# goroda/GPEXP

Hardware: AMD Instinct MI355X
Metric: GP-fit+IVAR-eval points/s at N=32768 d=8 (wall-time in ms_per_step); value = (N+M)/t_step, SURVEY 8d's N/t_fit and M/t_IVAR are points_per_s_fit / points_per_s_ivar right behind it (higher is better)
Workload: dtype f64; 1 GPU; C4: N=32768 d=8 Matern-5/2 (rho=0.5,s=1,noise=0.1) kfill+potrf+potrs+logdet+IVAR over M=32768 MC points; N=32768, d=8, M=32768, kernel=matern52, seed=32768, parallelism=1 GPU

## Files before the change

gpexp_amd/_lib.py:

```python
import ctypes as C
import os

import numpy as np

_HERE = os.path.dirname(os.path.abspath(__file__))
LIB_PATH = os.path.join(_HERE, "libgpx_hip.so")

c_i64 = C.c_int64
c_dp = C.POINTER(C.c_double)
c_ip = C.POINTER(c_i64)
c_vp = C.c_void_p

_SIGS = {
    "gpx_abi_version": (C.c_int, []),
    "gpx_last_error": (C.c_char_p, []),
    "gpx_create": (C.c_int, [C.c_int, C.POINTER(c_vp)]),
    "gpx_destroy": (C.c_int, [c_vp]),
    "gpx_sync": (C.c_int, [c_vp]),
    "gpx_trim": (C.c_int, [c_vp]),
    "gpx_device_info": (C.c_int, [c_vp, C.c_char_p, C.c_int, C.POINTER(C.c_int), c_ip, C.POINTER(C.c_int)]),
    "gpx_mat_from_host": (C.c_int, [c_vp, c_dp, c_i64, c_i64, C.c_int, C.POINTER(c_vp)]),
    "gpx_mat_alloc": (C.c_int, [c_vp, c_i64, c_i64, C.c_int, C.POINTER(c_vp)]),
    "gpx_mat_free": (C.c_int, [c_vp, c_vp]),
    "gpx_mat_clone": (C.c_int, [c_vp, c_vp, C.POINTER(c_vp)]),
    "gpx_mat_shape": (C.c_int, [c_vp, c_ip, c_ip, c_ip]),
    "gpx_mat_to_host": (C.c_int, [c_vp, c_vp, c_dp, C.c_int]),
    "gpx_kfill": (C.c_int, [c_vp, C.c_int, C.c_int, c_dp, C.c_int, c_vp, c_vp, c_dp, c_i64, C.POINTER(c_vp)]),
    "gpx_kfill_into": (C.c_int, [c_vp, C.c_int, C.c_int, c_dp, C.c_int, c_vp, c_vp, c_dp, c_i64, c_vp]),
    "gpx_kdiag": (C.c_int, [c_vp, C.c_int, C.c_int, c_dp, C.c_int, c_vp, c_dp]),
    "gpx_kernel_eval": (C.c_int, [c_vp, C.c_int, C.c_int, c_dp, C.c_int, c_dp, c_i64, c_dp, c_i64, c_dp]),
    "gpx_potrf": (C.c_int, [c_vp, c_vp]),
    "gpx_potrf_policy": (C.c_int, [c_vp, C.c_double, C.c_int]),
    "gpx_potrf_dropped": (C.c_int, [c_vp, C.POINTER(C.c_int)]),
    "gpx_refit_rows": (C.c_int, [c_vp, C.c_int, C.c_int, c_dp, C.c_int, c_vp, c_dp, c_i64, c_vp, c_i64, C.POINTER(c_vp)]),
    "gpx_potrs": (C.c_int, [c_vp, c_vp, c_dp, c_dp]),
    "gpx_col_sumsq": (C.c_int, [c_vp, c_vp, c_i64, c_dp]),
    "gpx_dist_ivar_step": (C.c_int, [c_vp, c_vp, c_i64, c_i64, c_vp]),
    "gpx_dist_ivar_group": (C.c_int, [c_vp, c_vp, c_i64, c_i64, c_i64, c_vp]),
    "gpx_dist_ivar_group_at": (C.c_int, [c_vp, c_vp, c_i64, c_i64, c_i64, c_vp, c_i64]),
    "gpx_dist_fwd_group_at": (C.c_int, [c_vp, c_vp, c_i64, c_i64, c_i64, c_vp, c_i64]),
    "gpx_matvec": (C.c_int, [c_vp, c_vp, c_dp, c_dp]),
    "gpx_fitc_fit": (C.c_int, [c_vp, C.c_int, C.c_int, c_dp, C.c_int, c_vp, c_vp, C.c_double, C.POINTER(c_vp)]),
    "gpx_fitc_free": (C.c_int, [c_vp, c_vp]),
    "gpx_fitc_shape": (C.c_int, [c_vp, C.POINTER(c_i64), C.POINTER(c_i64)]),
    "gpx_fitc_solve": (C.c_int, [c_vp, c_vp, c_dp, c_dp, c_dp]),
    "gpx_fitc_logdet": (C.c_int, [c_vp, c_vp, c_dp]),
    "gpx_fitc_posterior": (C.c_int, [c_vp, c_vp, c_vp, c_dp, c_vp, c_dp, c_dp]),
    "gpx_fitc_dense": (C.c_int, [c_vp, c_vp, c_dp, c_dp]),
    "gpx_potrs_dev": (C.c_int, [c_vp, c_vp, c_vp, c_vp]),
    "gpx_logdet": (C.c_int, [c_vp, c_vp, c_dp]),
    "gpx_potri": (C.c_int, [c_vp, c_vp, C.POINTER(c_vp)]),
    "gpx_posterior": (C.c_int, [c_vp, C.c_int, C.c_int, c_dp, C.c_int, c_vp, c_vp, c_dp, c_vp, c_dp, c_dp]),
    "gpx_posterior_cov": (C.c_int, [c_vp, C.c_int, C.c_int, c_dp, C.c_int, c_vp, c_vp, c_vp, c_dp]),
    "gpx_fit_ivar": (C.c_int, [c_vp, C.c_int, C.c_int, c_dp, C.c_int, c_vp, c_vp, c_vp, c_dp]),
    "gpx_ivar": (C.c_int, [c_vp, C.c_int, C.c_int, c_dp, C.c_int, c_vp, c_vp, c_vp, c_dp]),
    "gpx_ivar_keep": (C.c_int, [c_vp, C.c_int, C.c_int, c_dp, C.c_int, c_vp, c_vp, c_vp, c_dp, C.POINTER(c_vp)]),
    "gpx_ivar_update": (C.c_int, [c_vp, C.c_int, C.c_int, c_dp, C.c_int, c_vp, c_vp, c_vp, c_vp, c_i64, c_dp]),
    "gpx_greedy_var": (C.c_int, [c_vp, C.c_int, C.c_int, c_dp, C.c_int, c_vp, c_dp, c_ip, c_i64, c_i64, c_ip]),
    "gpx_greedy_ivar_step": (C.c_int, [c_vp, C.c_int, C.c_int, c_dp, C.c_int, c_vp, c_vp, c_vp, c_vp,
                                       C.c_double, c_dp, c_ip]),
    "gpx_greedy_ivar": (C.c_int, [c_vp, C.c_int, C.c_int, c_dp, C.c_int, c_vp, c_vp, c_vp, c_vp, C.c_double, c_i64, c_ip, c_dp,
                                  c_dp]),
    "gpx_givar_begin": (C.c_int, [c_vp, C.c_int, C.c_int, c_dp, C.c_int, c_vp, c_vp, c_vp, c_vp, C.c_double, c_i64,
                                  C.POINTER(c_vp)]),
    "gpx_givar_pivot_elems": (c_i64, [c_vp]),
    "gpx_givar_score": (C.c_int, [c_vp, c_vp, c_dp, c_ip, c_dp]),
    "gpx_givar_pack": (C.c_int, [c_vp, c_vp, c_i64, c_vp]),
    "gpx_givar_apply": (C.c_int, [c_vp, c_vp, c_vp]),
    "gpx_givar_end": (C.c_int, [c_vp, c_vp]),
    "gpx_mi_greedy": (C.c_int, [c_vp, C.c_int, C.c_int, c_dp, C.c_int, c_vp, C.c_double, c_i64, c_i64, c_ip, c_dp]),
    "gpx_acq": (C.c_int, [c_vp, C.c_int, C.c_int, c_dp, C.c_int, c_vp, c_vp, c_dp, c_vp, C.c_int, C.c_double, c_dp, c_ip, c_dp]),
    "gpx_acq_grad": (C.c_int, [c_vp, C.c_int, C.c_int, c_dp, C.c_int, c_vp, c_vp, c_dp, c_vp, C.c_int, C.c_double, c_dp, c_dp]),
    "gpx_acq_batch": (C.c_int, [c_vp, C.c_int, C.c_int, c_dp, C.c_int, c_vp, c_vp, c_dp, c_vp, C.c_double, C.c_int, C.c_double,
                                C.c_int, C.c_int, C.c_double, c_i64, c_ip, c_dp, c_dp, c_dp]),
    "gpx_lml_grad": (C.c_int, [c_vp, C.c_int, C.c_int, c_dp, C.c_int, c_vp, c_vp, c_dp, c_dp]),
    "gpx_lml_grad_slab": (C.c_int, [c_vp, C.c_int, C.c_int, c_dp, C.c_int, c_vp, c_vp, c_dp, c_i64, c_i64, c_dp]),
    "gpx_lml_grad_rows": (C.c_int, [c_vp, C.c_int, C.c_int, c_dp, C.c_int, c_vp, c_vp, c_dp, c_i64, c_i64, C.c_int, c_dp]),
    "gpx_lml_grad_linv": (C.c_int, [c_vp, C.c_int, C.c_int, c_dp, C.c_int, c_vp, c_vp, c_dp, c_dp]),
    "gpx_loo": (C.c_int, [c_vp, c_vp, c_dp, c_dp, c_dp, c_dp]),
    "gpx_loo_grad": (C.c_int, [c_vp, C.c_int, C.c_int, c_dp, C.c_int, c_vp, c_vp, c_dp, c_i64, c_dp, c_i64, c_dp, c_dp]),
    "gpx_mi_begin": (C.c_int, [c_vp, C.c_int, C.c_int, c_dp, C.c_int, c_vp, C.c_double, c_i64, c_i64, c_i64, c_i64, C.POINTER(c_vp)]),
    "gpx_mi_row": (C.c_int, [c_vp, c_vp, c_i64, c_i64, c_vp]),
    "gpx_mi_score": (C.c_int, [c_vp, c_vp, c_i64, c_vp, c_dp, c_ip]),
    "gpx_mi_select": (C.c_int, [c_vp, c_vp, c_i64, c_i64]),
    "gpx_mi_end": (C.c_int, [c_vp, c_vp]),
    "gpx_mat_read": (C.c_int, [c_vp, c_vp, c_i64, c_i64, c_dp]),
    "gpx_mat_write": (C.c_int, [c_vp, c_vp, c_i64, c_i64, c_dp]),
    "gpx_comm_unique_id": (C.c_int, [c_vp]),
    "gpx_comm_init": (C.c_int, [c_vp, C.c_int, C.c_int, c_vp]),
    "gpx_comm_destroy": (C.c_int, [c_vp]),
    "gpx_comm_bcast": (C.c_int, [c_vp, c_vp, c_i64, C.c_int]),
    "gpx_comm_allgather_host": (C.c_int, [c_vp, c_dp, c_i64, c_dp]),
    "gpx_dist_kfill": (C.c_int, [c_vp, C.c_int, C.c_int, c_dp, C.c_int, c_vp, c_dp, c_i64, c_vp, c_i64, C.c_int,
                                 C.c_int]),
    "gpx_dist_panel_elems": (c_i64, [c_i64, c_i64]),
    "gpx_dist_panel_factor": (C.c_int, [c_vp, c_vp, c_i64, c_i64, c_vp]),
    "gpx_dist_begin": (C.c_int, [c_vp]),
    "gpx_dist_info": (C.c_int, [c_vp, C.POINTER(C.c_int)]),
    "gpx_dist_panel_store": (C.c_int, [c_vp, c_vp, c_i64, c_i64, c_vp]),
    "gpx_dist_panel_update": (C.c_int, [c_vp, c_vp, c_i64, c_i64, c_vp, c_i64, c_i64, C.c_int, C.c_int]),
    "gpx_vec_op": (C.c_int, [c_vp, c_vp, c_i64, c_vp, c_i64, c_i64, C.c_int]),
    "gpx_comm_grid": (C.c_int, [c_vp, C.c_int, C.c_int]),
    "gpx_comm_bcast_grp": (C.c_int, [c_vp, c_vp, c_i64, c_i64, C.c_int, C.c_int]),
    "gpx_comm_bcast_grp2": (C.c_int, [c_vp, c_vp, c_i64, c_vp, c_i64, c_i64, C.c_int, C.c_int]),
    "gpx_comm_reduce_grp": (C.c_int, [c_vp, c_vp, c_i64, c_i64, C.c_int, C.c_int]),
    "gpx_comm_allreduce": (C.c_int, [c_vp, c_vp, c_i64, c_i64]),
    "gpx_comm_allreduce_host": (C.c_int, [c_vp, c_dp, c_i64]),
    "gpx_comm_panel_bcast": (C.c_int, [c_vp, c_vp, c_ip, c_ip, C.POINTER(C.c_int), C.c_int]),
    "gpx_dist2_diag_elems": (c_i64, [c_i64]),
    "gpx_dist2_row_stride": (c_i64, [c_i64]),
    "gpx_dist2_kfill": (C.c_int, [c_vp, C.c_int, C.c_int, c_dp, C.c_int, c_vp, c_dp, c_i64, c_vp, c_i64, C.c_int, C.c_int,
                                  C.c_int, C.c_int]),
    "gpx_dist2_diag_factor": (C.c_int, [c_vp, c_vp, c_i64, c_i64, c_i64, c_vp, c_i64, c_i64, c_i64, c_i64]),
    "gpx_dist2_diag_stage": (C.c_int, [c_vp, c_vp, c_i64, c_i64, c_i64, c_vp, c_i64, c_i64]),
    "gpx_dist2_diag_update": (C.c_int, [c_vp, c_vp, c_i64, c_i64, c_vp, c_i64, c_i64, c_i64]),
    "gpx_dist2_diag_factor_staged": (C.c_int, [c_vp, c_vp, c_i64, c_i64, c_i64, c_vp, c_i64, c_i64, c_i64, c_i64]),
    "gpx_dist2_diag_store": (C.c_int, [c_vp, c_vp, c_i64, c_i64, c_i64, c_vp, c_i64, c_i64, c_i64]),
    "gpx_dist2_reserve": (C.c_int, [c_vp, c_i64, c_i64, c_i64]),
    "gpx_dist2_panel_inv": (C.c_int, [c_vp, c_vp, c_i64, c_i64, c_i64]),
    "gpx_dist2_panel_trsm": (C.c_int, [c_vp, c_vp, c_i64, c_i64, c_i64, c_i64, c_vp, c_i64, c_i64, c_i64]),
    "gpx_dist2_panel_trsm_keep": (C.c_int, [c_vp, c_vp, c_i64, c_i64, c_i64, c_i64, c_vp, c_i64, c_i64, c_i64, c_i64]),
    "gpx_dist2_panel_trsm_inv": (C.c_int, [c_vp, c_vp, c_i64, c_i64, c_i64, c_i64, c_vp, c_i64, c_i64, c_i64, c_i64, C.c_int]),
    "gpx_dist2_panel_copyback": (C.c_int, [c_vp, c_vp, c_i64, c_i64, c_i64, c_i64, c_vp, c_i64, c_i64]),
    "gpx_points_set_box": (C.c_int, [c_vp, c_vp, c_dp, c_dp, C.c_int]),
    "gpx_dist2_panel_pack": (C.c_int, [c_vp, c_vp, c_i64, c_i64, c_i64, c_i64, c_vp, c_i64, c_i64]),
    "gpx_dist2_diag_pack": (C.c_int, [c_vp, c_vp, c_i64, c_i64, c_i64, c_vp, c_i64, c_i64]),
    "gpx_dist2_update": (C.c_int, [c_vp, c_vp, c_i64, c_i64, c_i64, c_i64, c_vp, c_i64, c_i64, c_i64, c_i64]),
    "gpx_dist2_update_multi": (C.c_int, [c_vp, c_vp, c_i64, c_i64, c_i64, c_i64, c_i64, C.c_int, C.c_int, C.c_int, C.c_int, c_i64,
                                         C.c_int, C.POINTER(c_vp), c_ip, C.c_int]),
    "gpx_dist2_pack_rows": (C.c_int, [c_vp, c_vp, c_i64, c_i64, c_i64, c_vp, c_i64, c_i64, c_i64, c_i64]),
    "gpx_dist2_pack_diag": (C.c_int, [c_vp, c_vp, c_i64, c_i64, c_i64, c_vp, c_i64]),
    "gpx_program_run": (C.c_int, [c_vp, c_ip, c_i64, c_ip, c_i64, c_dp]),
    "gpx_program_capture": (C.c_int, [c_vp, c_ip, c_i64, c_ip, c_i64, C.POINTER(c_vp)]),
    "gpx_graph_launch": (C.c_int, [c_vp, c_vp, c_dp, c_ip]),
    "gpx_graph_free": (C.c_int, [c_vp, c_vp]),
    "gpx_dist2_unpack_rows": (C.c_int, [c_vp, c_vp, c_i64, c_i64, c_i64, c_i64, c_vp, c_i64, c_i64, c_i64]),
    "gpx_dist2_unpack_diag": (C.c_int, [c_vp, c_vp, c_i64, c_i64, c_i64, c_vp, c_i64]),
    "gpx_dist2_unpack_diag_at": (C.c_int, [c_vp, c_vp, c_i64, c_i64, c_i64, c_vp, c_i64, c_i64]),
    "gpx_dist2_trsv_diag": (C.c_int, [c_vp, c_vp, c_i64, c_i64, c_i64, c_vp, c_i64, C.c_int]),
    "gpx_dist2_gemv": (C.c_int, [c_vp, c_vp, c_i64, c_i64, c_i64, c_i64, c_vp, c_i64, c_vp, c_i64, C.c_int]),
    "gpx_dist2_logdet_acc": (C.c_int, [c_vp, c_vp, c_i64, c_i64, c_i64, c_i64, c_vp]),
    "gpx_stream_select": (C.c_int, [c_vp, C.c_int]),
    "gpx_event_record": (C.c_int, [c_vp, C.c_int]),
    "gpx_event_wait": (C.c_int, [c_vp, C.c_int]),
    "gpx_dist_finish": (C.c_int, [c_vp, c_vp]),
    "gpx_ivar_grad": (C.c_int, [c_vp, C.c_int, C.c_int, c_dp, C.c_int, c_vp, c_vp, c_vp, c_dp, c_dp]),
    "gpx_ivar_grad_w": (C.c_int, [c_vp, C.c_int, C.c_int, c_dp, C.c_int, c_vp, c_vp, c_vp, c_dp, c_vp, c_dp]),
    "gpx_ivar_grad_rows": (C.c_int, [c_vp, C.c_int, C.c_int, c_dp, C.c_int, c_vp, c_vp, c_vp, c_vp, c_i64, c_dp]),
    "gpx_var_grad": (C.c_int, [c_vp, C.c_int, C.c_int, c_dp, C.c_int, c_vp, c_vp, c_vp, c_dp, c_dp, c_dp, c_dp]),
    "gpx_var_grad_newpt": (C.c_int, [c_vp, C.c_int, C.c_int, c_dp, C.c_int, c_vp, c_vp, c_vp, c_dp]),
    "gpx_fitc_var_grad": (C.c_int, [c_vp, c_vp, C.c_int, C.c_int, c_dp, C.c_int, c_vp, c_vp, c_dp, c_dp, c_dp, c_dp]),
    "gpx_fitc_var_grad_newpt": (C.c_int, [c_vp, c_vp, C.c_int, C.c_int, c_dp, C.c_int, c_vp, c_vp, c_dp]),
    "gpx_profile_enable": (C.c_int, [c_vp, C.c_int]),
    "gpx_profile_reset": (C.c_int, [c_vp]),
    "gpx_profile_get": (C.c_int, [c_vp, C.c_int, c_ip, c_dp, c_dp, c_dp]),
    "gpx_dbg_gemm": (C.c_int, [c_vp, c_vp, c_vp, c_vp, C.c_int, C.c_int, C.c_int]),
    "gpx_dbg_gemm_strassen": (C.c_int, [c_vp, c_vp, c_vp, c_vp]),
    "gpx_dbg_gemm_strassen_depth": (C.c_int, [c_vp, c_vp, c_vp, c_vp, C.c_int]),
    "gpx_dbg_gemm_tri": (C.c_int, [c_vp, c_vp, c_vp, c_vp, C.c_int, C.c_int, C.c_int]),
    "gpx_dbg_gemm_ksplit": (C.c_int, [c_vp, c_vp, c_vp, c_vp, C.c_int, C.c_int]),
    "gpx_dbg_kfill_plan": (C.c_int, [c_vp, C.c_int, C.c_int, c_dp, C.c_int, c_vp, c_vp, C.POINTER(C.c_int), c_dp]),
    "gpx_dbg_colreduce_plan": (C.c_int, [c_i64, c_i64, C.POINTER(c_i64), C.POINTER(c_i64)]),
    "gpx_dbg_panel_bcast_plan": (C.c_int, [C.c_int, C.c_int, c_i64, C.c_int, C.POINTER(c_i64), C.POINTER(C.c_int),
                                           C.POINTER(c_i64), c_i64, C.POINTER(c_i64)]),
    "gpx_dbg_guard_violations": (c_i64, [c_vp]),
    "gpx_dbg_guard_selftest": (C.c_int, [c_vp]),
    "gpx_dbg_spin": (C.c_int, [c_vp, C.c_int]),
    "gpx_dbg_spin_us": (C.c_int, [c_vp, c_i64]),
    "gpx_dbg_stamp": (C.c_int, [c_vp, C.c_int]),
    "gpx_dbg_spin_until": (C.c_int, [c_vp, C.c_int, c_i64]),
    "gpx_dbg_event_elapsed": (C.c_int, [c_vp, C.c_int, C.c_int, c_dp]),
    "gpx_dbg_leaf_stamps": (C.c_int, [c_vp, c_vp, C.c_int, C.POINTER(c_i64)]),
}

_lib = None


def load():
    global _lib
    if _lib is not None:
        return _lib
    path = os.environ.get("GPX_LIB_PATH", LIB_PATH)
    if not os.path.exists(path):
        raise ImportError(
            "gpexp_amd: %s not found - the HIP library is required (no CPU fallback). "
            "Build it with `make -C gpexp_amd/csrc` or __graft_entry__.build()." % path)
    lib = C.CDLL(path)
    for name, (res, args) in _SIGS.items():
        fn = getattr(lib, name)
        fn.restype = res
        fn.argtypes = args
    if lib.gpx_abi_version() != 2:
        raise ImportError("gpexp_amd: libgpx_hip.so ABI version mismatch")
    _lib = lib
    return lib


def hdot(a, b):
    import numpy as _np
    return float(_np.sum(_np.multiply(a, b)))


def exported_symbols():
    return sorted(_SIGS)


class GpxError(RuntimeError):
    pass


class NotPositiveDefinite(GpxError):
    def __init__(self, pivot):
        super().__init__("covariance matrix is not positive definite: pivot %d <= 0 "
                         "(the reference's pinv would silently truncate here, gp.py:181)" % pivot)
        self.pivot = pivot


def check(rc):
    if rc == 0:
        return
    if rc > 0:
        raise NotPositiveDefinite(rc)
    raise GpxError("libgpx_hip: " + load().gpx_last_error().decode("utf-8", "replace"))


def as_f64(a):
    return np.ascontiguousarray(a, dtype=np.float64)


def dptr(a):
    return a.ctypes.data_as(c_dp) if a is not None else None
```

gpexp_amd/csrc/api.hip:

```cpp
#include "gpx_internal.h"
#include <stdarg.h>
#include <stdio.h>
#include <string.h>
#include <math.h>
#include <stdlib.h>

static thread_local char g_err[1024] = "";

void gpx_set_error(const char* fmt, ...) {
  va_list ap;
  va_start(ap, fmt);
  vsnprintf(g_err, sizeof(g_err), fmt, ap);
  va_end(ap);
}

static constexpr int64_t GUARD = 4096;

int gpx_dev_alloc(gpx_ctx* ctx, int64_t bytes, void** out) {
  if (bytes <= 0) bytes = 8;
  bytes = gpx_round_up(bytes, 256);
  const int64_t key = bytes + (ctx->guard ? 2 * GUARD : 0);
  void* base = nullptr;
  auto it = ctx->pool.find(key);
  if (it != ctx->pool.end()) {
    base = it->second;
    ctx->pool.erase(it);
    ctx->pool_bytes -= key;
    auto pf = ctx->pending.find(base);
    if (pf != ctx->pending.end()) {
      for (hipEvent_t ev : pf->second->evs) (void)hipEventSynchronize(ev);
      if (pf->second.use_count() == 1)
        for (hipEvent_t ev : pf->second->evs) ctx->fence_free.push_back(ev);
      ctx->pending.erase(pf);
    }
  } else {
    hipError_t e = hipMalloc(&base, (size_t)key);
    if (e != hipSuccess) {
      (void)hipGetLastError();
      gpx_trim(ctx);
      e = hipMalloc(&base, (size_t)key);
    }
    if (e != hipSuccess) {
      gpx_set_error("hipMalloc(%lld bytes) failed: %s", (long long)key, hipGetErrorString(e));
      return -2;
    }
  }
  if (ctx->guard) {
    GPX_HIP(hipDeviceSynchronize());
    GPX_HIP(hipMemset(base, 0xA5, (size_t)GUARD));
    GPX_HIP(hipMemset((char*)base + GUARD + bytes, 0xA5, (size_t)GUARD));
    if (ctx->guard >= 2) GPX_HIP(hipMemset((char*)base + GUARD, 0xFF, (size_t)bytes));
    GPX_HIP(hipDeviceSynchronize());
    *out = (char*)base + GUARD;
  } else {
    *out = base;
  }
  return 0;
}

void gpx_dev_release(gpx_ctx* ctx, void* p, int64_t bytes) {
  if (!p) return;
  if (bytes <= 0) bytes = 8;
  bytes = gpx_round_up(bytes, 256);
  const int64_t key = bytes + (ctx->guard ? 2 * GUARD : 0);
  void* base = p;
  if (ctx->guard) {
    base = (char*)p - GUARD;
    std::vector<unsigned char> h((size_t)(2 * GUARD));
    (void)hipDeviceSynchronize();
    if (hipMemcpy(h.data(), base, (size_t)GUARD, hipMemcpyDeviceToHost) == hipSuccess &&
        hipMemcpy(h.data() + GUARD, (char*)p + bytes, (size_t)GUARD, hipMemcpyDeviceToHost) == hipSuccess) {
      int64_t below = 0, above = 0;
      for (int64_t i = 0; i < GUARD; ++i) {
        below += h[(size_t)i] != 0xA5;
        above += h[(size_t)(GUARD + i)] != 0xA5;
      }
      if (below || above) {
        ctx->guard_violations += 1;
        fprintf(stderr, "gpx: ALLOCATION GUARD VIOLATED: %lld-byte block, %lld bytes overwritten below, %lld above\n",
                (long long)bytes, (long long)below, (long long)above);
      }
    }
  }
  ctx->pool.insert({key, base});
  ctx->pool_bytes += key;
}

__global__ void dbg_spin_kernel(long long ticks) {
  const long long t0 = wall_clock64();
  while (wall_clock64() - t0 < ticks) {}
}

static double spin_ticks_per_us(gpx_ctx* ctx) {
  static double tpu = 0.0;
  if (tpu == 0.0) {
    int khz = 0;
    if (hipDeviceGetAttribute(&khz, hipDeviceAttributeWallClockRate, ctx->device) != hipSuccess || khz <= 0) {
      (void)hipGetLastError();
      khz = 100000;
    }
    tpu = (double)khz / 1000.0;
  }
  return tpu;
}

ProfScope::ProfScope(gpx_ctx* c, int cls, double flops, double bytes) : ctx(c), idx(-1) {
  if (c->chaos) {
    c->chaos = c->chaos * 6364136223846793005ULL + 1442695040888963407ULL;
    const unsigned r = (unsigned)(c->chaos >> 33);
    if ((r & 3u) == 0u)
      hipLaunchKernelGGL(dbg_spin_kernel, dim3(1), dim3(64), 0, c->stream,
                         (long long)((100.0 + (double)((r >> 2) % 2900)) * spin_ticks_per_us(c)));
  }
  if (!c->prof_on) return;
  c->prof_launches[cls] += 1;
  c->prof_flops[cls] += flops;
  c->prof_bytes[cls] += bytes;
  if (!c->prof_recs.empty()) {
    ProfRec& last = c->prof_recs.back();
    if (last.cls == cls && last.stream == c->stream && !last.open) {
      last.open = true;
      idx = (int)c->prof_recs.size() - 1;
      return;
    }
  }
  ProfRec r;
  r.cls = cls;
  r.stream = c->stream;
  r.open = true;
  hipEvent_t ev[2];
  for (int i = 0; i < 2; ++i) {
    if (!c->ev_free.empty()) {
      ev[i] = c->ev_free.back();
      c->ev_free.pop_back();
    } else if (hipEventCreate(&ev[i]) != hipSuccess) {
      return;
    }
  }
  r.a = ev[0];
  r.b = ev[1];
  (void)hipEventRecord(r.a, c->stream);
  c->prof_recs.push_back(r);
  idx = (int)c->prof_recs.size() - 1;
}

ProfScope::~ProfScope() {
  if (idx >= 0) {
    ProfRec& r = ctx->prof_recs[(size_t)idx];
    (void)hipEventRecord(r.b, r.stream);
    r.open = false;
  }
}

int gpx_prof_flush(gpx_ctx* ctx) {
  if (ctx->prof_recs.empty()) return 0;
  GPX_HIP(hipDeviceSynchronize());
  for (auto& r : ctx->prof_recs) {
    float ms = 0.f;
    if (hipEventElapsedTime(&ms, r.a, r.b) == hipSuccess) ctx->prof_ms[r.cls] += ms;
    ctx->ev_free.push_back(r.a);
    ctx->ev_free.push_back(r.b);
  }
  ctx->prof_recs.clear();
  return 0;
}

int gpx_make_kparams(int kind, int d, const double* hyp, int nhyp, KParams* kp) {
  GPX_ARG(d >= 1 && d <= GPX_MAXD, "dimension must be in [1, GPX_MAX_DIM]");
  GPX_ARG(hyp != nullptr, "hyp is NULL");
  memset(kp, 0, sizeof(*kp));
  kp->kind = kind;
  kp->d = d;
  switch (kind) {
    case GPX_K_SE:
      GPX_ARG(nhyp == d + 1, "SE needs d correlation lengths + signalSize");
      for (int k = 0; k < d; ++k) kp->scale[k] = 1.0 / hyp[k];
      kp->sig = hyp[d];
      break;
    case GPX_K_MATERN32:
    case GPX_K_MATERN52: {
      GPX_ARG(nhyp == 2, "Matern needs {rho, signalSize}");
      const double c = (kind == GPX_K_MATERN32 ? sqrt(3.0) : sqrt(5.0)) / hyp[0];
      for (int k = 0; k < d; ++k) kp->scale[k] = c;
      kp->sig = hyp[1];
      break;
    }
    case GPX_K_MEHLER: {
      GPX_ARG(nhyp == d, "Mehler needs d parameters t_k");
      double s = 1.0;
      for (int k = 0; k < d; ++k) {
        const double t = hyp[k], om = 1.0 - t * t;
        kp->scale[k] = 1.0;
        kp->c1[k] = t * t / (2.0 * om);
        kp->c2[k] = t / om;
        s *= pow(om, -0.5);
      }
      kp->sig = s;
      break;
    }
    default: gpx_set_error("unknown kernel kind %d", kind); return -1;
  }
  return 0;
}

static void bbox_from_host(gpx_mat* m, const double* src, int64_t rows, int64_t cols, int64_t ld) {
  m->bbox_ok = 0;
  m->bad_row = m->bad_col = -1;
  if (cols < 1 || cols > GPX_MAXD || rows < 1) return;
  for (int64_t k = 0; k < cols; ++k) m->lo[k] = m->hi[k] = src[k];
  for (int64_t i = 0; i < rows; ++i) {
    const double* r = src + i * ld;
    for (int64_t k = 0; k < cols; ++k) {
      const double v = r[k];
      if (v < m->lo[k]) m->lo[k] = v;
      if (v > m->hi[k]) m->hi[k] = v;
      if (!(fabs(v) <= 1.79769313486231570815e308) && m->bad_row < 0) {
        m->bad_row = i;
        m->bad_col = k;
      }
    }
  }
  m->bbox_ok = 1;
}

static int mat_bbox(gpx_ctx* ctx, const gpx_mat* cm) {
  gpx_mat* m = const_cast<gpx_mat*>(cm);
  if (m->bbox_ok || m->rows < 1) return 0;
  GPX_ARG(m->cols >= 1 && m->cols <= GPX_MAXD, "point set has more than GPX_MAX_DIM columns");
  std::vector<double> h((size_t)(m->rows * m->cols));
  GPX_HIP(hipMemcpy2DAsync(h.data(), (size_t)m->cols * 8, m->p, (size_t)m->ld * 8, (size_t)m->cols * 8, (size_t)m->rows,
                           hipMemcpyDeviceToHost, ctx->stream));
  GPX_HIP(hipStreamSynchronize(ctx->stream));
  bbox_from_host(m, h.data(), m->rows, m->cols, m->cols);
  return 0;
}

extern "C" int gpx_points_set_box(gpx_ctx* ctx, gpx_mat* P, const double* lo, const double* hi, int d) {
  GPX_ARG(ctx && P && lo && hi && d >= 1 && d <= GPX_MAXD && P->cols == d, "points_set_box: bad arguments");
  GPX_TRY(mat_bbox(ctx, P));
  for (int k = 0; k < d; ++k) {
    GPX_ARG(lo[k] <= hi[k], "points_set_box: empty box");
    P->lo[k] = lo[k];
    P->hi[k] = hi[k];
  }
  P->bbox_ok = 1;
  return 0;
}

static double exact_threshold() {
  const char* e = getenv("GPX_EXACT_S");
  return e ? atof(e) : 120.0;
}

int gpx_kparams_sets(gpx_ctx* ctx, KParams* kp, const gpx_mat* A, const gpx_mat* B, const gpx_mat* C) {
  for (int k = 0; k < GPX_MAXD; ++k) kp->center[k] = 0.0;
  kp->exact = 0;
  const gpx_mat* sets[3] = {A, B, C};
  double lo[GPX_MAXD], hi[GPX_MAXD];
  bool any = false;
  for (const gpx_mat* s : sets) {
    if (!s || s->rows < 1) continue;
    GPX_TRY(mat_bbox(ctx, s));
    if (s->bad_row >= 0) {
      gpx_set_error("point set has a non-finite coordinate (NaN or infinity) at row %lld, column %lld",
                    (long long)s->bad_row, (long long)s->bad_col);
      return -1;
    }
    if (kp->kind == GPX_K_MEHLER) continue;
    for (int k = 0; k < kp->d; ++k) {
      if (!any || s->lo[k] < lo[k]) lo[k] = s->lo[k];
      if (!any || s->hi[k] > hi[k]) hi[k] = s->hi[k];
    }
    any = true;
  }
  if (!any || kp->kind == GPX_K_MEHLER) return 0;
  double S = 0.0;
  for (int k = 0; k < kp->d; ++k) {
    const double c = 0.5 * lo[k] + 0.5 * hi[k];
    kp->center[k] = fabs(c) < 1e300 ? c : 0.0;
    const double hw = (hi[k] - kp->center[k]) * kp->scale[k];
    S += 2.0 * hw * hw;
  }
  const double sens = kp->kind == GPX_K_MATERN52 ? 1.0 / 6.0 : 0.5;
  kp->exact = !(S * sens <= exact_threshold());
  return 0;
}

__global__ __launch_bounds__(256) static void sub_partials_kernel(const double* __restrict__ P, int64_t nbat, int64_t n,
                                                                  double* __restrict__ C, int64_t ldc) {
  const int64_t j = (int64_t)blockIdx.x * 256 + threadIdx.x, i = blockIdx.y;
  if (j >= n || j > i) return;
  double s = 0.0;
  for (int64_t b = 0; b < nbat; ++b) s += P[(b * n + i) * n + j];
  C[i * ldc + j] -= s;
}

int launch_sub_partials(gpx_ctx* ctx, const double* P, int64_t nbat, int64_t n, double* C, int64_t ldc) {
  hipLaunchKernelGGL(sub_partials_kernel, dim3((unsigned)((n + 255) / 256), (unsigned)n), dim3(256), 0, ctx->stream, P, nbat, n, C,
                     ldc);
  GPX_HIP(hipGetLastError());
  return 0;
}

int gpx_mat_new(gpx_ctx* ctx, int64_t rows, int64_t cols, int pad, gpx_mat** out) {
  GPX_ARG(rows >= 0 && cols >= 0, "negative shape");
  gpx_mat* m = new gpx_mat();
  m->rows = rows;
  m->cols = cols;
  m->prows = pad ? gpx_round_up(rows > 0 ? rows : 1, GPX_TILE) : (rows > 0 ? rows : 1);
  m->pcols = pad ? gpx_round_up(cols > 0 ? cols : 1, GPX_TILE) : (cols > 0 ? cols : 1);
  m->ld = pad ? gpx_skew_ld(m->pcols) : m->pcols;
  m->bytes = m->prows * m->ld * (int64_t)sizeof(double);
  m->aux = nullptr;
  m->aux_bytes = 0;
  m->factored = 0;
  m->bbox_ok = 0;
  m->bad_row = m->bad_col = -1;
  m->binv = nullptr;
  m->binv_bytes = 0;
// ... 37 lines not shown
  for (int i = 0; i < 3; ++i) {
    c->grp[i] = nullptr;
    c->grp_size[i] = 1;
    c->grp_rank[i] = 0;
  }
  c->Pr = c->Pc = 1;
  c->piv_min = 0.0;
  c->piv_skip = 0;
  c->pw_binv = c->pw_tmp_build = c->pw_tmp_T = nullptr;
  c->pw_ib = 0;
  c->pw_done = 0;
  c->prof_on = 0;
  for (int i = 0; i < GPX_PROF_NCLASS; ++i) {
    c->prof_launches[i] = 0;
    c->prof_ms[i] = c->prof_flops[i] = c->prof_bytes[i] = 0.0;
  }
  {
    int lo = 0, hi = 0;
    GPX_HIP(hipDeviceGetStreamPriorityRange(&lo, &hi));
    const int mainp = (lo - hi >= 2) ? (lo + hi) / 2 : lo;
    GPX_HIP(hipStreamCreateWithPriority(&c->streams[0], hipStreamNonBlocking, mainp));
    GPX_HIP(hipStreamCreateWithPriority(&c->streams[1], hipStreamNonBlocking, hi));
    GPX_HIP(hipStreamCreateWithPriority(&c->streams[2], hipStreamNonBlocking, hi));
    GPX_HIP(hipStreamCreateWithPriority(&c->streams[4], hipStreamNonBlocking, lo));
    c->stream = c->streams[0];
  }
  hipDeviceProp_t prop;
  GPX_HIP(hipGetDeviceProperties(&prop, device));
  c->cus = prop.multiProcessorCount;
  {
    const int words = (c->cus + 31) / 32;
    std::vector<uint32_t> mask((size_t)words, 0xffffffffu);
    if (c->cus % 32) mask[(size_t)words - 1] = (1u << (c->cus % 32)) - 1u;
    for (int cu = 0; cu < 4; ++cu)
      for (int x = 0; x < 8; ++x) {
        const int bit = 8 * cu + x;
        if (bit < c->cus) mask[(size_t)bit / 32] &= ~(1u << (bit % 32));
      }
    for (int si : {3, 5}) {
      if (words < 2 || hipExtStreamCreateWithCUMask(&c->streams[si], (uint32_t)words, mask.data()) != hipSuccess) {
        (void)hipGetLastError();
        int lo = 0, hi = 0;
        GPX_HIP(hipDeviceGetStreamPriorityRange(&lo, &hi));
        GPX_HIP(hipStreamCreateWithPriority(&c->streams[si], hipStreamNonBlocking, lo));
      }
    }
  }
  GPX_HIP(hipMalloc((void**)&c->d_info, 256));
  GPX_HIP(hipMalloc((void**)&c->d_scal, 64 * sizeof(double)));
  GPX_HIP(hipMemset(c->d_info, 0, 256));
  c->trsv_scratch = nullptr;
  c->trsv_scratch_bytes = 0;
  c->d2_scratch = nullptr;
  c->dbg_stamps = nullptr;
  c->d2_scratch_bytes = 0;
  c->d2_inv_src = nullptr;
  c->d2_inv_nb = 0;
  c->ev_scratch = nullptr;
  c->ev_scratch_bytes = 0;
  *out = c;
  return 0;
}

int gpx_dbg_spin(gpx_ctx* ctx, int ms) {
  GPX_ARG(ctx && ms >= 0 && ms <= 500, "spin: 0..500 ms");
  if (ms == 0) return 0;
  hipLaunchKernelGGL(dbg_spin_kernel, dim3(1), dim3(64), 0, ctx->stream, (long long)((double)ms * 1000.0 * spin_ticks_per_us(ctx)));
  GPX_HIP(hipGetLastError());
  return 0;
}

int gpx_dbg_spin_us(gpx_ctx* ctx, int64_t us) {
  GPX_ARG(ctx && us >= 0 && us <= 500000, "spin: 0..500000 us");
  if (us == 0) return 0;
  hipLaunchKernelGGL(dbg_spin_kernel, dim3(1), dim3(64), 0, ctx->stream, (long long)((double)us * spin_ticks_per_us(ctx)));
  GPX_HIP(hipGetLastError());
  return 0;
}

constexpr int GPX_DBG_STAMPS = 1024;
__global__ void dbg_stamp_kernel(long long* slot) { *slot = wall_clock64(); }
__global__ void dbg_spin_until_kernel(const long long* slot, long long ticks, long long cap) {
  const long long t0 = wall_clock64(), target = *slot + ticks;
  while (wall_clock64() < target && wall_clock64() - t0 < cap) {}
}
static int dbg_stamps_ensure(gpx_ctx* ctx) {
  if (!ctx->dbg_stamps) {
    GPX_HIP(hipMalloc((void**)&ctx->dbg_stamps, GPX_DBG_STAMPS * sizeof(long long)));
    GPX_HIP(hipMemset(ctx->dbg_stamps, 0, GPX_DBG_STAMPS * sizeof(long long)));
  }
  return 0;
}
int gpx_dbg_stamp(gpx_ctx* ctx, int slot) {
  GPX_ARG(ctx && slot >= 0 && slot < GPX_DBG_STAMPS, "stamp: slot 0..1023");
  GPX_TRY(dbg_stamps_ensure(ctx));
  hipLaunchKernelGGL(dbg_stamp_kernel, dim3(1), dim3(1), 0, ctx->stream, ctx->dbg_stamps + slot);
  GPX_HIP(hipGetLastError());
  return 0;
}
int gpx_dbg_spin_until(gpx_ctx* ctx, int slot, int64_t us) {
  GPX_ARG(ctx && slot >= 0 && slot < GPX_DBG_STAMPS && us <= 500000, "spin_until: slot 0..1023, at most 500000 us");
  if (us <= 0) return 0;
  GPX_TRY(dbg_stamps_ensure(ctx));
  hipLaunchKernelGGL(dbg_spin_until_kernel, dim3(1), dim3(1), 0, ctx->stream, ctx->dbg_stamps + slot,
                     (long long)((double)us * spin_ticks_per_us(ctx)), (long long)(500000.0 * spin_ticks_per_us(ctx)));
  GPX_HIP(hipGetLastError());
  return 0;
}

int64_t gpx_dbg_guard_violations(gpx_ctx* ctx) { return ctx ? (ctx->guard ? ctx->guard_violations : -1) : -1; }

int gpx_dbg_guard_selftest(gpx_ctx* ctx) {
  GPX_ARG(ctx && ctx->guard, "guard mode is off");
  void* p;
  GPX_TRY(gpx_dev_alloc(ctx, 1024, &p));
  GPX_HIP(hipMemset((char*)p + 1024, 0, 16));
  const int64_t before = ctx->guard_violations;
  gpx_dev_release(ctx, p, 1024);
  const int caught = ctx->guard_violations == before + 1;
  ctx->guard_violations = before;
  return caught;
}

int gpx_trim(gpx_ctx* ctx) {
  GPX_ARG(ctx != nullptr, "ctx is NULL");
  (void)hipDeviceSynchronize();
  for (auto& kv : ctx->pending)
    if (kv.second.use_count() == 1)
      for (hipEvent_t ev : kv.second->evs) ctx->fence_free.push_back(ev);
  ctx->pending.clear();
  for (auto& kv : ctx->pool) (void)hipFree(kv.second);
  ctx->pool.clear();
  ctx->pool_bytes = 0;
  return 0;
}

int gpx_destroy(gpx_ctx* ctx) {
  if (!ctx) return 0;
  (void)hipSetDevice(ctx->device);
  gpx_comm_destroy(ctx);
  gpx_prof_flush(ctx);
  gpx_trim(ctx);
  for (auto ev : ctx->ev_free) (void)hipEventDestroy(ev);
  for (auto ev : ctx->fence_free) (void)hipEventDestroy(ev);
  (void)hipFree(ctx->d_info);
  (void)hipFree(ctx->d_scal);
  if (ctx->trsv_scratch) (void)hipFree(ctx->trsv_scratch);
  if (ctx->d2_scratch) (void)hipFree(ctx->d2_scratch);
  if (ctx->dbg_stamps) (void)hipFree(ctx->dbg_stamps);
  if (ctx->ev_scratch) (void)hipFree(ctx->ev_scratch);
  for (auto ev : ctx->sync_events) (void)hipEventDestroy(ev);
  for (auto ev : ctx->la_events) (void)hipEventDestroy(ev);
  if (ctx->ev_side) (void)hipEventDestroy(ctx->ev_side);
  for (int i = 0; i < GPX_NSTREAMS; ++i) {
    bool seen = false;
    for (int j = 0; j < i; ++j) seen = seen || ctx->streams[j] == ctx->streams[i];
    if (!seen) (void)hipStreamDestroy(ctx->streams[i]);
  }
  delete ctx;
  return 0;
}

int gpx_sync(gpx_ctx* ctx) {
  GPX_ARG(ctx != nullptr, "ctx is NULL");
  GPX_HIP(hipSetDevice(ctx->device));
  GPX_HIP(hipDeviceSynchronize());
  return 0;
}

int gpx_stream_select(gpx_ctx* ctx, int which) {
  GPX_ARG(ctx && which >= 0 && which < GPX_NSTREAMS,
          "stream index must be 0 (main), 1 (panel), 2 (communication), 3 (background, CU-masked), 4 (evaluation) or 5 (bulk, "
          "CU-masked)");
  ctx->stream = ctx->streams[which];
  return 0;
}

static int sync_event(gpx_ctx* ctx, int id, hipEvent_t* out) {
  GPX_ARG(ctx && id >= 0 && id < 65536, "event id out of range");
  while ((int)ctx->sync_events.size() <= id) {
    hipEvent_t ev;
    static int timing = -1;
    if (timing < 0) timing = getenv("GPX_EVENT_TIMING") ? atoi(getenv("GPX_EVENT_TIMING")) : 0;
    GPX_HIP(hipEventCreateWithFlags(&ev, timing ? hipEventDefault : hipEventDisableTiming));
    ctx->sync_events.push_back(ev);
  }
  *out = ctx->sync_events[(size_t)id];
  return 0;
}

int gpx_dbg_event_elapsed(gpx_ctx* ctx, int id0, int id1, double* ms) {
  GPX_ARG(ctx && ms && id0 >= 0 && id1 >= 0, "bad arguments");
  if (id0 >= (int)ctx->sync_events.size() || id1 >= (int)ctx->sync_events.size()) return 1;
  float f = 0.0f;
  if (hipEventElapsedTime(&f, ctx->sync_events[(size_t)id0], ctx->sync_events[(size_t)id1]) != hipSuccess) {
    (void)hipGetLastError();
    return 1;
  }
  *ms = (double)f;
  return 0;
}

int gpx_event_record(gpx_ctx* ctx, int id) {
  hipEvent_t ev;
  GPX_TRY(sync_event(ctx, id, &ev));
  GPX_HIP(hipEventRecord(ev, ctx->stream));
  return 0;
}

int gpx_event_wait(gpx_ctx* ctx, int id) {
  hipEvent_t ev;
  GPX_TRY(sync_event(ctx, id, &ev));
  GPX_HIP(hipStreamWaitEvent(ctx->stream, ev, 0));
  return 0;
}

int gpx_device_info(gpx_ctx* ctx, char* name, int name_len, int* cus, int64_t* hbm_bytes, int* clock_mhz) {
  GPX_ARG(ctx != nullptr, "ctx is NULL");
  hipDeviceProp_t prop;
  GPX_HIP(hipGetDeviceProperties(&prop, ctx->device));
  if (name && name_len > 0) {
    snprintf(name, (size_t)name_len, "%s (%s)", prop.name, prop.gcnArchName);
  }
  if (cus) *cus = prop.multiProcessorCount;
  if (hbm_bytes) *hbm_bytes = (int64_t)prop.totalGlobalMem;
  if (clock_mhz) *clock_mhz = prop.clockRate / 1000;
  return 0;
}

int gpx_mat_alloc(gpx_ctx* ctx, int64_t rows, int64_t cols, int pad, gpx_mat** out) {
  GPX_ARG(ctx && out, "NULL argument");
  GPX_TRY(gpx_mat_new(ctx, rows, cols, pad, out));
  GPX_HIP(hipMemsetAsync((*out)->p, 0, (size_t)(*out)->bytes, ctx->stream));
  GPX_HIP(hipStreamSynchronize(ctx->stream));
  return 0;
}

int gpx_mat_from_host(gpx_ctx* ctx, const double* src, int64_t rows, int64_t cols, int pad, gpx_mat** out) {
  GPX_ARG(ctx && out && (src || rows * cols == 0), "NULL argument");
  GPX_TRY(gpx_mat_alloc(ctx, rows, cols, pad, out));
  gpx_mat* m = *out;
  if (rows > 0 && cols > 0)
    GPX_HIP(hipMemcpy2DAsync(m->p, (size_t)m->ld * 8, src, (size_t)cols * 8, (size_t)cols * 8, (size_t)rows,
                             hipMemcpyHostToDevice, ctx->stream));
  if (!pad) bbox_from_host(m, src, rows, cols, cols);
  GPX_HIP(hipStreamSynchronize(ctx->stream));
  return 0;
}

int gpx_mat_clone(gpx_ctx* ctx, const gpx_mat* src, gpx_mat** out) {
  GPX_ARG(ctx && src && out, "NULL argument");
  const int padded = src->prows != (src->rows > 0 ? src->rows : 1) || src->pcols != (src->cols > 0 ? src->cols : 1) ||
                     src->ld != src->pcols;
  GPX_TRY(gpx_mat_new(ctx, src->rows, src->cols, padded, out));
  gpx_mat* m = *out;
  if (m->bytes != src->bytes || m->ld != src->ld) {
    gpx_mat_free(ctx, m);
    *out = nullptr;
    GPX_ARG(false, "clone: storage layout of the copy differs from the source");
  }
  auto fail = [&](const char* what) {
    gpx_set_error("clone: %s failed: %s", what, hipGetErrorString(hipGetLastError()));
    gpx_mat_free(ctx, m);
    *out = nullptr;
    return -2;
  };
  if (hipMemcpyAsync(m->p, src->p, (size_t)src->bytes, hipMemcpyDeviceToDevice, ctx->stream) != hipSuccess) return fail("copy");
  if (src->aux) {
    void* p = nullptr;
    int r = gpx_dev_alloc(ctx, src->aux_bytes, &p);
    if (r != 0) {
      gpx_mat_free(ctx, m);
      *out = nullptr;
      return r;
    }
    m->aux = (double*)p;
    m->aux_bytes = src->aux_bytes;
    if (hipMemcpyAsync(m->aux, src->aux, (size_t)src->aux_bytes, hipMemcpyDeviceToDevice, ctx->stream) != hipSuccess)
      return fail("copy of the leaf inverses");
  }
  m->factored = src->factored;
  m->bbox_ok = src->bbox_ok;
  m->bad_row = src->bad_row;
  m->bad_col = src->bad_col;
  for (int k = 0; k < GPX_MAXD; ++k) {
    m->lo[k] = src->lo[k];
    m->hi[k] = src->hi[k];
  }
  if (hipStreamSynchronize(ctx->stream) != hipSuccess) return fail("synchronisation");
  return 0;
}

int gpx_mat_free(gpx_ctx* ctx, gpx_mat* m) {
  if (!m) return 0;
  GPX_ARG(ctx != nullptr, "ctx is NULL");
  if (ctx->guard) {
    (void)hipDeviceSynchronize();
  } else {
    auto f = std::make_shared<gpx_ctx::Fence>();
    bool ok = true;
    for (int i = 0; i < GPX_NSTREAMS && ok; ++i) {
      hipEvent_t ev = nullptr;
      if (!ctx->fence_free.empty()) {
        ev = ctx->fence_free.back();
        ctx->fence_free.pop_back();
      } else if (hipEventCreateWithFlags(&ev, hipEventDisableTiming) != hipSuccess) {
// ... 366 lines not shown
  return 0;
}

static int need_factor(const gpx_mat* L) {
  GPX_ARG(L != nullptr, "factor is NULL");
  GPX_ARG(L->factored && L->aux, "matrix has not been factored by gpx_potrf");
  return 0;
}

int gpx_potrs(gpx_ctx* ctx, const gpx_mat* L, const double* y, double* alpha) {
  GPX_ARG(ctx && y && alpha, "NULL argument");
  GPX_TRY(need_factor(L));
  const int64_t n = L->rows, np = L->prows;
  const int64_t sb = chol_potrs_scratch_bytes(np);
  void *p, *ps;
  GPX_TRY(gpx_dev_alloc(ctx, np * 8, &p));
  int r = gpx_dev_alloc(ctx, sb, &ps);
  if (r != 0) {
    gpx_dev_release(ctx, p, np * 8);
    return r;
  }
  double* dv = (double*)p;
  do {
    if (hipMemsetAsync(dv, 0, (size_t)np * 8, ctx->stream) != hipSuccess) { r = -2; break; }
    if (hipMemcpyAsync(dv, y, (size_t)n * 8, hipMemcpyHostToDevice, ctx->stream) != hipSuccess) { r = -2; break; }
    if ((r = chol_potrs(ctx, const_cast<gpx_mat*>(L), dv, (double*)ps)) != 0) break;
    if (hipMemcpyAsync(alpha, dv, (size_t)n * 8, hipMemcpyDeviceToHost, ctx->stream) != hipSuccess) { r = -2; break; }
  } while (0);
  (void)hipStreamSynchronize(ctx->stream);
  gpx_dev_release(ctx, dv, np * 8);
  gpx_dev_release(ctx, ps, sb);
  if (r == -2) gpx_set_error("potrs: HIP copy failed");
  return r;
}

int gpx_potrs_dev(gpx_ctx* ctx, const gpx_mat* L, const gpx_mat* y, gpx_mat* alpha) {
  GPX_ARG(ctx && y && alpha, "NULL argument");
  GPX_TRY(need_factor(L));
  const int64_t np = L->prows;
  GPX_ARG(y->bytes >= np * 8 && alpha->bytes >= np * 8, "y / alpha must hold the padded length (zero padded)");
  const int64_t need = chol_potrs_scratch_bytes(np);
  if (ctx->trsv_scratch_bytes < need) {
    GPX_HIP(hipDeviceSynchronize());
    if (ctx->trsv_scratch) (void)hipFree(ctx->trsv_scratch);
    ctx->trsv_scratch = nullptr;
    ctx->trsv_scratch_bytes = 0;
    GPX_HIP(hipMalloc((void**)&ctx->trsv_scratch, (size_t)need));
    ctx->trsv_scratch_bytes = need;
  }
  if (alpha->p != y->p)
    GPX_HIP(hipMemcpyAsync(alpha->p, y->p, (size_t)np * 8, hipMemcpyDeviceToDevice, ctx->stream));
  return chol_potrs(ctx, const_cast<gpx_mat*>(L), alpha->p, ctx->trsv_scratch);
}

int gpx_logdet(gpx_ctx* ctx, const gpx_mat* L, double* out) {
  GPX_ARG(ctx && out, "NULL argument");
  GPX_TRY(need_factor(L));
  GPX_TRY(launch_logdet(ctx, L->p, L->ld, L->rows, ctx->d_scal));
  GPX_HIP(hipMemcpyAsync(out, ctx->d_scal, 8, hipMemcpyDeviceToHost, ctx->stream));
  GPX_HIP(hipStreamSynchronize(ctx->stream));
  return 0;
}

__global__ __launch_bounds__(256) static void vec_diff_kernel(const double* __restrict__ a, const double* __restrict__ b,
                                                              int64_t n, double* __restrict__ out) {
  const int64_t j = (int64_t)blockIdx.x * 256 + threadIdx.x;
  if (j < n) out[j] = a[j] - b[j];
}

__global__ __launch_bounds__(1024) static void pairwise_mean_kernel(double* __restrict__ v, int64_t count,
                                                                     double* __restrict__ out) {
  int64_t m = count;
  while (m > 1) {
    const int64_t h = (m + 1) / 2;
    for (int64_t i = threadIdx.x; i + h < m; i += 1024) v[i] += v[i + h];
    __syncthreads();
    m = h;
  }
  if (threadIdx.x == 0) out[0] = v[0] / (double)count;
}

static int64_t eval_chunk(int64_t np) {
  int64_t budget = (int64_t)16 << 30;
  const char* e = getenv("GPX_CROSS_BYTES");
  if (e && atoll(e) > 0) budget = atoll(e);
  int64_t mc = budget / (np * 8) / GPX_TILE * GPX_TILE;
  if (mc < GPX_TILE) mc = GPX_TILE;
  return mc;
}
int64_t gpx_eval_chunk(int64_t np) { return eval_chunk(np); }

static int posterior_impl(gpx_ctx* ctx, const KParams& kp, const gpx_mat* L, const gpx_mat* X, const double* alpha,
                          const gpx_mat* Z, double* mean, double* var_host, double* var_dev = nullptr,
                          gpx_mat** keepW = nullptr) {
  const int64_t n = L->rows, np = L->prows, M = Z->rows, d = kp.d;
  const bool var = var_host != nullptr || var_dev != nullptr;
  if (keepW) *keepW = nullptr;
  GPX_ARG(X->rows == n, "X does not match the factor");
  if (M == 0) return 0;
  const int64_t mcmax = eval_chunk(np);
  const int64_t mc_alloc = gpx_round_up(M < mcmax ? M : mcmax, GPX_TILE);
  void *pB = nullptr, *pW = nullptr, *pal = nullptr, *pout = nullptr, *ppart = nullptr, *pkd = nullptr;
  const bool oop = var && np >= 2048;
  const int64_t ldb_alloc = gpx_skew_ld(mc_alloc);
  const int64_t bytesB = np * ldb_alloc * 8, bytes_out = mc_alloc * 8;
  const int64_t bytes_part = colreduce_partial_elems(np, mc_alloc) * 8 + 8;
  int r = 0;
  void* pvar = nullptr;
  do {
    if (var && !var_dev) {
      if ((r = gpx_dev_alloc(ctx, M * 8, &pvar)) != 0) break;
      var_dev = (double*)pvar;
    }
    gpx_mat* Wm = nullptr;
    if (keepW && var && M <= mcmax && gpx_mat_new(ctx, n, M, 1, &Wm) == 0 &&
        (Wm->prows != np || Wm->ld != ldb_alloc || Wm->bytes < bytesB)) {
      gpx_mat_free(ctx, Wm);
      Wm = nullptr;
    }
    if (Wm) *keepW = Wm;
    if (Wm && !oop) pB = Wm->p;
    else if ((r = gpx_dev_alloc(ctx, bytesB, &pB)) != 0) break;
    if (oop) {
      if (Wm) pW = Wm->p;
      else if ((r = gpx_dev_alloc(ctx, bytesB, &pW)) != 0) break;
    }
    if ((r = gpx_dev_alloc(ctx, bytes_out, &pout)) != 0) break;
    if ((r = gpx_dev_alloc(ctx, bytes_out, &pkd)) != 0) break;
    if ((r = gpx_dev_alloc(ctx, bytes_part, &ppart)) != 0) break;
    if (mean) {
      if ((r = gpx_dev_alloc(ctx, np * 8, &pal)) != 0) break;
      if (hipMemsetAsync(pal, 0, (size_t)np * 8, ctx->stream) != hipSuccess ||
          hipMemcpyAsync(pal, alpha, (size_t)n * 8, hipMemcpyHostToDevice, ctx->stream) != hipSuccess) {
        r = -2;
        break;
      }
    }
    for (int64_t j0 = 0; j0 < M && r == 0; j0 += mcmax) {
      const int64_t mc = (M - j0) < mcmax ? (M - j0) : mcmax;
      const int64_t mcp = gpx_round_up(mc, GPX_TILE);
      double* B = (double*)pB;
      const double* Zc = Z->p + j0 * d;
      const int64_t ldb = gpx_skew_ld(mcp);
      if ((r = launch_kfill(ctx, kp, X->p, n, Zc, mc, 0, nullptr, 0, 0.0, B, np, mcp, ldb)) != 0) break;
      if (mean) {
        if ((r = launch_colreduce(ctx, B, ldb, n, mcp, (const double*)pal, (double*)pout, (double*)ppart)) != 0) break;
        if (hipMemcpyAsync(mean + j0, pout, (size_t)mc * 8, hipMemcpyDeviceToHost, ctx->stream) != hipSuccess) {
          r = -2;
          break;
        }
      }
      if (var) {
        const double* Wsol = B;
        if (oop) {
          if ((r = chol_trsm_left_oop(ctx, const_cast<gpx_mat*>(L), B, ldb, (double*)pW, ldb, mcp)) != 0) break;
          Wsol = (const double*)pW;
        } else if ((r = chol_trsm_left(ctx, L->p, L->ld, L->aux, B, ldb, np, mcp)) != 0) {
          break;
        }
        if ((r = launch_colreduce(ctx, Wsol, ldb, n, mcp, nullptr, (double*)pout, (double*)ppart)) != 0) break;
        if ((r = launch_kdiag(ctx, kp, Zc, mc, (double*)pkd)) != 0) break;
        hipLaunchKernelGGL(vec_diff_kernel, dim3((unsigned)((mc + 255) / 256)), dim3(256), 0, ctx->stream, (const double*)pkd,
                           (const double*)pout, mc, var_dev + j0);
      }
    }
    if (r == 0 && var_host &&
        hipMemcpyAsync(var_host, var_dev, (size_t)M * 8, hipMemcpyDeviceToHost, ctx->stream) != hipSuccess)
      r = -2;
  } while (0);
  (void)hipStreamSynchronize(ctx->stream);
  if (pvar) gpx_dev_release(ctx, pvar, M * 8);
  {
    gpx_mat* Wm = keepW ? *keepW : nullptr;
    if (pB && !(Wm && pB == (void*)Wm->p)) gpx_dev_release(ctx, pB, bytesB);
    if (pW && !(Wm && pW == (void*)Wm->p)) gpx_dev_release(ctx, pW, bytesB);
    if (Wm && r != 0) {
      gpx_mat_free(ctx, Wm);
      *keepW = nullptr;
    }
  }
  gpx_dev_release(ctx, pout, bytes_out);
  gpx_dev_release(ctx, pkd, bytes_out);
  gpx_dev_release(ctx, ppart, bytes_part);
  if (pal) gpx_dev_release(ctx, pal, np * 8);
  if (r == -2) gpx_set_error("posterior: HIP copy failed: %s", hipGetErrorString(hipGetLastError()));
  return r;
}

int gpx_posterior(gpx_ctx* ctx, int kind, int d, const double* hyp, int nhyp, const gpx_mat* L, const gpx_mat* X,
                  const double* alpha, const gpx_mat* Z, double* mean, double* var) {
  GPX_ARG(ctx && X && Z, "NULL argument");
  GPX_TRY(need_factor(L));
  GPX_ARG(mean == nullptr || alpha != nullptr, "alpha is required for the mean");
  KParams kp;
  GPX_TRY(gpx_make_kparams(kind, d, hyp, nhyp, &kp));
  GPX_ARG(X->cols == d && X->pcols == d && Z->cols == d && Z->pcols == d, "point sets must be unpadded (n x d)");
  GPX_TRY(gpx_kparams_sets(ctx, &kp, X, Z));
  return posterior_impl(ctx, kp, L, X, alpha, Z, mean, var);
}

static double pairwise_mean(std::vector<double>& v, int64_t count) {
  int64_t m = count;
  while (m > 1) {
    int64_t h = (m + 1) / 2;
    for (int64_t i = 0; i + h < m; ++i) v[(size_t)i] += v[(size_t)(i + h)];
    m = h;
  }
  return v[0] / (double)count;
}

static int ivar_impl(gpx_ctx* ctx, int kind, int d, const double* hyp, int nhyp, const gpx_mat* L, const gpx_mat* X,
                     const gpx_mat* Z, double* out, gpx_mat** W);

int gpx_ivar(gpx_ctx* ctx, int kind, int d, const double* hyp, int nhyp, const gpx_mat* L, const gpx_mat* X,
             const gpx_mat* Z, double* out) {
  return ivar_impl(ctx, kind, d, hyp, nhyp, L, X, Z, out, nullptr);
}

int gpx_ivar_keep(gpx_ctx* ctx, int kind, int d, const double* hyp, int nhyp, const gpx_mat* L, const gpx_mat* X,
                  const gpx_mat* Z, double* out, gpx_mat** W) {
  GPX_ARG(W != nullptr, "W is NULL");
  return ivar_impl(ctx, kind, d, hyp, nhyp, L, X, Z, out, W);
}

static int ivar_impl(gpx_ctx* ctx, int kind, int d, const double* hyp, int nhyp, const gpx_mat* L, const gpx_mat* X,
                     const gpx_mat* Z, double* out, gpx_mat** W) {
  GPX_ARG(ctx && X && Z && out, "NULL argument");
  if (W) *W = nullptr;
  GPX_TRY(need_factor(L));
  KParams kp;
  GPX_TRY(gpx_make_kparams(kind, d, hyp, nhyp, &kp));
  GPX_ARG(X->cols == d && X->pcols == d && Z->cols == d && Z->pcols == d, "point sets must be unpadded (n x d)");
  GPX_ARG(Z->rows > 0, "IVAR needs at least one integration point");
  GPX_TRY(gpx_kparams_sets(ctx, &kp, X, Z));
  void* pv;
  GPX_TRY(gpx_dev_alloc(ctx, Z->rows * 8, &pv));
  int r = posterior_impl(ctx, kp, L, X, nullptr, Z, nullptr, nullptr, (double*)pv, W);
  if (r == 0) {
    hipLaunchKernelGGL(pairwise_mean_kernel, dim3(1), dim3(1024), 0, ctx->stream, (double*)pv, Z->rows, ctx->d_scal);
    if (hipMemcpyAsync(out, ctx->d_scal, 8, hipMemcpyDeviceToHost, ctx->stream) != hipSuccess) r = -2;
  }
  (void)hipStreamSynchronize(ctx->stream);
  gpx_dev_release(ctx, pv, Z->rows * 8);
  if (r == -2) gpx_set_error("ivar: HIP copy failed");
  if (r != 0 && W && *W) {
    gpx_mat_free(ctx, *W);
    *W = nullptr;
  }
  return r;
}

int gpx_ivar_update(gpx_ctx* ctx, int kind, int d, const double* hyp, int nhyp, const gpx_mat* L, const gpx_mat* X,
                    const gpx_mat* Z, gpx_mat* W, int64_t keep, double* out) {
  GPX_ARG(ctx && X && Z && W && out, "NULL argument");
  GPX_TRY(need_factor(L));
  GPX_ARG(ctx->live_mats.count(W), "ivar_update: W is not a live matrix of this context");
  KParams kp;
  GPX_TRY(gpx_make_kparams(kind, d, hyp, nhyp, &kp));
  GPX_ARG(X->cols == d && X->pcols == d && Z->cols == d && Z->pcols == d, "point sets must be unpadded (n x d)");
  const int64_t n = L->rows, np = L->prows, M = Z->rows, mcp = gpx_round_up(M, GPX_TILE);
  GPX_ARG(X->rows == n && M > 0, "X does not match the factor / no integration points");
  GPX_ARG(W->rows == n && W->cols == M && W->prows == np && W->pcols == mcp, "ivar_update: W has another shape");
  GPX_ARG(keep > 0 && keep < np && keep % GPX_TILE == 0, "ivar_update: keep must be a positive multiple of 128 below the padded order");
  GPX_TRY(gpx_kparams_sets(ctx, &kp, X, Z));
  const int64_t n2 = n - keep, n2p = np - keep, ldw = W->ld;
  const int64_t bytes_out = mcp * 8, bytes_part = colreduce_partial_elems(np, mcp) * 8 + 8;
  void *pout = nullptr, *pkd = nullptr, *ppart = nullptr, *pv = nullptr;
  int r = 0;
  do {
    if ((r = gpx_dev_alloc(ctx, bytes_out, &pout)) != 0) break;
    if ((r = gpx_dev_alloc(ctx, bytes_out, &pkd)) != 0) break;
    if ((r = gpx_dev_alloc(ctx, bytes_part, &ppart)) != 0) break;
    if ((r = gpx_dev_alloc(ctx, M * 8, &pv)) != 0) break;
    double* W2 = W->p + keep * ldw;
    if ((r = launch_kfill(ctx, kp, X->p + keep * d, n2, Z->p, M, 0, nullptr, 0, 0.0, W2, n2p, mcp, ldw)) != 0) break;
    if ((r = launch_gemm(ctx, L->p + keep * L->ld, L->ld, W->p, ldw, W2, ldw, n2p, mcp, keep, false, true, false)) != 0) break;
    if ((r = chol_trsm_left(ctx, L->p + keep * (L->ld + 1), L->ld, L->aux + (keep / GPX_TILE) * GPX_TILE * GPX_TILE, W2, ldw, n2p,
                            mcp)) != 0) break;
    if ((r = launch_colreduce(ctx, W->p, ldw, n, mcp, nullptr, (double*)pout, (double*)ppart)) != 0) break;
    if ((r = launch_kdiag(ctx, kp, Z->p, M, (double*)pkd)) != 0) break;
    hipLaunchKernelGGL(vec_diff_kernel, dim3((unsigned)((M + 255) / 256)), dim3(256), 0, ctx->stream, (const double*)pkd,
                       (const double*)pout, M, (double*)pv);
    hipLaunchKernelGGL(pairwise_mean_kernel, dim3(1), dim3(1024), 0, ctx->stream, (double*)pv, M, ctx->d_scal);
    if (hipMemcpyAsync(out, ctx->d_scal, 8, hipMemcpyDeviceToHost, ctx->stream) != hipSuccess) r = -2;
  } while (0);
  (void)hipStreamSynchronize(ctx->stream);
  if (pout) gpx_dev_release(ctx, pout, bytes_out);
  if (pkd) gpx_dev_release(ctx, pkd, bytes_out);
  if (ppart) gpx_dev_release(ctx, ppart, bytes_part);
  if (pv) gpx_dev_release(ctx, pv, M * 8);
  if (r == -2) gpx_set_error("ivar_update: HIP copy failed");
  return r;
}

int gpx_fit_ivar(gpx_ctx* ctx, int kind, int d, const double* hyp, int nhyp, gpx_mat* K, const gpx_mat* X, const gpx_mat* Z,
                 double* out) {
  GPX_ARG(ctx && K && X && Z && out, "NULL argument");
  KParams kp;
  GPX_TRY(gpx_make_kparams(kind, d, hyp, nhyp, &kp));
  GPX_ARG(X->cols == d && X->pcols == d && Z->cols == d && Z->pcols == d, "point sets must be unpadded (n x d)");
  GPX_ARG(K->rows == X->rows && Z->rows > 0, "K does not match X / IVAR needs at least one integration point");
  GPX_ARG(ctx->stream == ctx->streams[0], "gpx_fit_ivar runs from the main stream");
  GPX_TRY(gpx_kparams_sets(ctx, &kp, X, Z));
  const int64_t M = Z->rows;
  PotrfJob J;
  GPX_TRY(potrf_begin(ctx, K, &J));
  int info = potrf_end(ctx, K, &J);
  if (info != 0) return info;
  std::vector<double> var((size_t)M);
  GPX_TRY(posterior_impl(ctx, kp, K, X, nullptr, Z, nullptr, var.data()));
  *out = pairwise_mean(var, M);
  return 0;
}

int gpx_col_sumsq(gpx_ctx* ctx, const gpx_mat* B, int64_t rows, double* out) {
  GPX_ARG(ctx && B && out && rows >= 0 && rows <= B->prows, "bad arguments");
  void *po, *pp;
  const int64_t bytes_part = colreduce_partial_elems(B->prows, B->pcols) * 8 + 8;
  GPX_TRY(gpx_dev_alloc(ctx, B->pcols * 8, &po));
  int r = gpx_dev_alloc(ctx, bytes_part, &pp);
  if (r == 0) {
    r = launch_colreduce(ctx, B->p, B->ld, rows, B->pcols, nullptr, (double*)po, (double*)pp);
    if (r == 0 && hipMemcpyAsync(out, po, (size_t)B->cols * 8, hipMemcpyDeviceToHost, ctx->stream) != hipSuccess) r = -2;
    (void)hipStreamSynchronize(ctx->stream);
    gpx_dev_release(ctx, pp, bytes_part);
  }
  gpx_dev_release(ctx, po, B->pcols * 8);
  if (r == -2) gpx_set_error("col_sumsq: HIP copy failed");
  return r;
}

int gpx_matvec(gpx_ctx* ctx, const gpx_mat* A, const double* v, double* out) {
  GPX_ARG(ctx && A && v && out, "NULL argument");
  GPX_ARG(A->pcols % 2 == 0 && A->ld % 2 == 0, "matvec needs an even padded width");
  void *pv, *po;
  GPX_TRY(gpx_dev_alloc(ctx, A->pcols * 8, &pv));
  int r = gpx_dev_alloc(ctx, (A->rows > 0 ? A->rows : 1) * 8, &po);
  if (r == 0) {
    do {
      if (hipMemsetAsync(pv, 0, (size_t)A->pcols * 8, ctx->stream) != hipSuccess ||
          hipMemcpyAsync(pv, v, (size_t)A->cols * 8, hipMemcpyHostToDevice, ctx->stream) != hipSuccess) { r = -2; break; }
      if ((r = launch_rowreduce(ctx, A->p, A->ld, A->rows, A->pcols, (const double*)pv, (double*)po)) != 0) break;
      if (hipMemcpyAsync(out, po, (size_t)A->rows * 8, hipMemcpyDeviceToHost, ctx->stream) != hipSuccess) { r = -2; break; }
    } while (0);
    (void)hipStreamSynchronize(ctx->stream);
    gpx_dev_release(ctx, po, (A->rows > 0 ? A->rows : 1) * 8);
  }
  gpx_dev_release(ctx, pv, A->pcols * 8);
  if (r == -2) gpx_set_error("matvec: HIP copy failed");
  return r;
}

int gpx_profile_enable(gpx_ctx* ctx, int on) {
  GPX_ARG(ctx != nullptr, "ctx is NULL");
  if (!on) GPX_TRY(gpx_prof_flush(ctx));
  ctx->prof_on = on ? 1 : 0;
  return 0;
}

int gpx_profile_reset(gpx_ctx* ctx) {
  GPX_ARG(ctx != nullptr, "ctx is NULL");
  GPX_TRY(gpx_prof_flush(ctx));
  for (int i = 0; i < GPX_PROF_NCLASS; ++i) {
    ctx->prof_launches[i] = 0;
    ctx->prof_ms[i] = ctx->prof_flops[i] = ctx->prof_bytes[i] = 0.0;
  }
  return 0;
}

int gpx_profile_get(gpx_ctx* ctx, int cls, int64_t* launches, double* ms, double* flops, double* bytes) {
  GPX_ARG(ctx != nullptr, "ctx is NULL");
  GPX_ARG(cls >= 0 && cls < GPX_PROF_NCLASS, "unknown profile class");
  GPX_TRY(gpx_prof_flush(ctx));
  if (launches) *launches = ctx->prof_launches[cls];
  if (ms) *ms = ctx->prof_ms[cls];
  if (flops) *flops = ctx->prof_flops[cls];
  if (bytes) *bytes = ctx->prof_bytes[cls];
  return 0;
}

int gpx_dbg_gemm_tri(gpx_ctx* ctx, const gpx_mat* A, const gpx_mat* B, gpx_mat* C, int bt, int accumulate, int tri) {
  GPX_ARG(ctx && A && B && C, "NULL argument");
  const int64_t m = C->prows, n = C->pcols, k = A->pcols;
  GPX_ARG(A->prows == m, "A rows");
  GPX_ARG(bt ? (B->prows == n && B->pcols == k) : (B->prows == k && B->pcols == n), "B shape");
  GPX_TRY(launch_gemm_tri(ctx, A->p, A->ld, B->p, B->ld, C->p, C->ld, m, n, k, bt != 0, accumulate != 0, tri == 3, tri));
  GPX_HIP(hipStreamSynchronize(ctx->stream));
  return 0;
}

int gpx_dbg_kfill_plan(gpx_ctx* ctx, int kind, int d, const double* hyp, int nhyp, const gpx_mat* X, const gpx_mat* Z,
                       int* exact, double* center) {
  GPX_ARG(ctx && X && exact && center, "NULL argument");
  KParams kp;
  GPX_TRY(gpx_make_kparams(kind, d, hyp, nhyp, &kp));
  GPX_TRY(gpx_kparams_sets(ctx, &kp, X, Z));
  *exact = kp.exact;
  for (int k = 0; k < d; ++k) center[k] = kp.center[k];
  return 0;
}

int gpx_dbg_gemm_ksplit(gpx_ctx* ctx, const gpx_mat* A, const gpx_mat* B, gpx_mat* C, int mode, int parts) {
  GPX_ARG(ctx && A && B && C && mode >= 0 && mode <= 3 && parts > 0, "bad argument");
  const int64_t m = C->prows, n = C->pcols, k = A->pcols;
  GPX_ARG(A->prows == m && B->prows == n && B->pcols == k, "operand shapes");
  void* P;
  const int64_t pb = (int64_t)parts * m * n * 8;
  GPX_TRY(gpx_dev_alloc(ctx, pb, &P));
  int r = mode <= 1 ? launch_gemm_ksplit(ctx, A->p, A->ld, B->p, B->ld, C->p, C->ld, m, n, k, mode == 1, parts, (double*)P)
                    : launch_gemm_ksplit_small(ctx, A->p, A->ld, B->p, B->ld, C->p, C->ld, m, n, k, mode == 3, parts, (double*)P);
  (void)hipStreamSynchronize(ctx->stream);
  gpx_dev_release(ctx, P, pb);
  return r;
}

int gpx_dbg_gemm(gpx_ctx* ctx, const gpx_mat* A, const gpx_mat* B, gpx_mat* C, int bt, int accumulate, int lower) {
  GPX_ARG(ctx && A && B && C, "NULL argument");
  const int64_t m = C->prows, n = C->pcols, k = A->pcols;
  GPX_ARG(A->prows == m, "A rows");
  GPX_ARG(bt ? (B->prows == n && B->pcols == k) : (B->prows == k && B->pcols == n), "B shape");
  GPX_TRY(launch_gemm(ctx, A->p, A->ld, B->p, B->ld, C->p, C->ld, m, n, k, bt != 0, accumulate != 0,
                      lower != 0));
  GPX_HIP(hipStreamSynchronize(ctx->stream));
  return 0;
}

int gpx_dbg_gemm_strassen(gpx_ctx* ctx, const gpx_mat* A, const gpx_mat* B, gpx_mat* C) {
  GPX_ARG(ctx && A && B && C, "NULL argument");
  const int64_t m = C->prows, n = C->pcols, k = A->pcols;
  GPX_ARG(A->prows == m && B->prows == k && B->pcols == n, "operand shapes");
  GPX_TRY(launch_gemm_strassen(ctx, A->p, A->ld, B->p, B->ld, C->p, C->ld, m, n, k, 1, nullptr, 0));
  GPX_HIP(hipStreamSynchronize(ctx->stream));
  return 0;
}

int gpx_dbg_gemm_strassen_depth(gpx_ctx* ctx, const gpx_mat* A, const gpx_mat* B, gpx_mat* C, int depth) {
  GPX_ARG(ctx && A && B && C, "NULL argument");
  GPX_ARG(depth >= 0 && depth <= GPX_STRASSEN_MAX_DEPTH, "strassen: depth out of range");
  const int64_t m = C->prows, n = C->pcols, k = A->pcols;
  GPX_ARG(A->prows == m && B->prows == k && B->pcols == n, "operand shapes");
  GPX_TRY(launch_gemm_strassen(ctx, A->p, A->ld, B->p, B->ld, C->p, C->ld, m, n, k, depth, nullptr, 0));
  GPX_HIP(hipStreamSynchronize(ctx->stream));
  return 0;
}

}
```

gpexp_amd/csrc/chol.hip:

```cpp
#include "gpx_internal.h"
#include <algorithm>
#include <math.h>
#include <stdlib.h>
#include <stddef.h>

namespace {

constexpr int NB = GPX_TILE;
constexpr int LS = NB + 1;

typedef double d4 __attribute__((ext_vector_type(4)));

__device__ __forceinline__ double readlane_d(double v, int srclane) {
  int lo = __builtin_amdgcn_readlane(__double2loint(v), srclane);
  int hi = __builtin_amdgcn_readlane(__double2hiint(v), srclane);
  return __hiloint2double(hi, lo);
}

constexpr int LB = 16;
constexpr int TS17 = LB + 1;
constexpr int BSZ = LB * TS17;
constexpr int LEAF_CB = LB * LB + 64 + LB;

__device__ __forceinline__ constexpr int sb_off(int I, int J) { return (I * (I + 1) / 2 + J) * BSZ; }
// ... 1050 lines not shown
  return trsv_fwd_rec(ctx, L + n1 * ld + n1, ld, invd + (n1 / NB) * NB * NB, y + n1, n2);
}

static int trsv_bwd_rec(gpx_ctx* ctx, const double* L, int64_t ld, const double* invd, double* z, int64_t n,
                        double* tmp, double* part) {
  if (n <= TRSV_BLOCK) {
    hipLaunchKernelGGL(trsv_block_bwd_kernel, dim3(1), dim3(256), 0, ctx->stream, L, ld, invd, z, (int)(n / NB));
    return 0;
  }
  const int64_t n1 = split(n), n2 = n - n1;
  GPX_TRY(trsv_bwd_rec(ctx, L + n1 * ld + n1, ld, invd + (n1 / NB) * NB * NB, z + n1, n2, tmp, part));
  GPX_TRY(launch_colreduce(ctx, L + n1 * ld, ld, n2, n1, z + n1, z, part, 1));
  return trsv_bwd_rec(ctx, L, ld, invd, z, n1, tmp, part);
}


static int64_t potrs_block(int64_t n) {
  int64_t ib = 1024;
  if (ib > n) ib = n;
  return ib;
}

static int binv_build_rec(gpx_ctx* ctx, const double* L, int64_t ld, int64_t sl, double* binv, int64_t ib, int64_t r0,
                          int64_t sz, double* tmp, int64_t batch, int64_t lo = 0, int64_t hi = INT64_MAX) {
  if (sz <= NB || sz <= lo) return 0;
  const int64_t s1 = split(sz), s2 = sz - s1;
  GPX_TRY(binv_build_rec(ctx, L, ld, sl, binv, ib, r0, s1, tmp, batch, lo, hi));
  GPX_TRY(binv_build_rec(ctx, L, ld, sl, binv, ib, r0 + s1, s2, tmp, batch, lo, hi));
  if (sz > hi) return 0;
  const double* C = L + (r0 + s1) * ld + r0;
  const double* Ai = binv + r0 * ib + r0;
  const double* Bi = binv + (r0 + s1) * ib + r0 + s1;
  double* R = binv + (r0 + s1) * ib + r0;
  if (batch == 1 && s1 >= 1024) {
    GPX_TRY(launch_gemm_tri(ctx, C, ld, Ai, ib, tmp, s1, s2, s1, s1, false, false, false, 4));
    return launch_gemm_tri(ctx, Bi, ib, tmp, s1, R, ib, s2, s1, s2, false, true, false, 1);
  }
  GPX_TRY(launch_gemm_batched(ctx, C, ld, sl, Ai, ib, ib * ib, tmp, s1, ib * ib, s2, s1, s1, false, false, batch));
  return launch_gemm_batched(ctx, Bi, ib, ib * ib, tmp, s1, ib * ib, R, ib, ib * ib, s2, s1, s2, false, true, batch);
}

static int binv_build_levels(gpx_ctx* ctx, const double* L, int64_t ld, double* binv, int64_t ib, int64_t w, double* tmp,
                             int64_t lo, int64_t hi) {
  for (int64_t sz = 2 * NB; sz <= w; sz *= 2) {
    if (sz <= lo) continue;
    if (sz > hi) break;
    const int64_t s1 = sz / 2, nbat = w / sz, sl = sz * (ld + 1), sb = sz * (ib + 1);
    GPX_TRY(launch_gemm_batched(ctx, L + s1 * ld, ld, sl, binv, ib, sb, tmp, s1, s1 * s1, s1, s1, s1, false, false, nbat));
    GPX_TRY(launch_gemm_batched(ctx, binv + s1 * (ib + 1), ib, sb, tmp, s1, s1 * s1, binv + s1 * ib, ib, sb, s1, s1, s1, false, true,
                                nbat));
  }
  return 0;
}

static int binv_build_range(gpx_ctx* ctx, const double* Ld, int64_t ld, const double* invd, double* binv, int64_t ib, int64_t n,
                            double* tmp, int64_t lo, int64_t hi) {
  const int64_t nblk = (n + ib - 1) / ib, nfull = n / ib, tail = n - nfull * ib;
  const int64_t rows = nblk * ib;
  if (lo == 0)
    hipLaunchKernelGGL(binv_init_kernel, dim3((unsigned)((rows * (ib / 2) + 255) / 256)), dim3(256), 0, ctx->stream, invd, binv,
                       ib, n);
  if (nfull == 1 && tail == 0 && ib <= 1024 && ((ib / NB) & (ib / NB - 1)) == 0) {
    GPX_TRY(binv_build_levels(ctx, Ld, ld, binv, ib, ib, tmp, lo, hi));
    GPX_HIP(hipGetLastError());
    return 0;
  }
  if (nfull > 0) GPX_TRY(binv_build_rec(ctx, Ld, ld, ib * (ld + 1), binv, ib, 0, ib, tmp, nfull, lo, hi));
  if (tail > 0)
    GPX_TRY(binv_build_rec(ctx, Ld + nfull * ib * (ld + 1), ld, 0, binv + nfull * ib * ib, ib, 0, tail, tmp, 1, lo, hi));
  GPX_HIP(hipGetLastError());
  return 0;
}

int chol_block_inverse(gpx_ctx* ctx, const double* D, int64_t ldd, const double* invd, double* inv, int64_t w, double* tmp) {
  GPX_ARG(w > 0 && w % NB == 0, "block inverse: order must be a positive multiple of 128");
  return binv_build_range(ctx, D, ldd, invd, inv, w, w, tmp);
}

int chol_trtri(gpx_ctx* ctx, const gpx_mat* Lm, double* Linv, double* tmp) {
  const int64_t n = Lm->prows;
  hipLaunchKernelGGL(binv_init_kernel, dim3((unsigned)((n * (n / 2) + 255) / 256)), dim3(256), 0, ctx->stream, Lm->aux, Linv, n, n);
  GPX_HIP(hipGetLastError());
  if (n >= 2048 && ((n / NB) & (n / NB - 1)) == 0) {
    GPX_TRY(binv_build_levels(ctx, Lm->p, Lm->ld, Linv, n, n, tmp, 0, 1024));
    return binv_build_rec(ctx, Lm->p, Lm->ld, 0, Linv, n, 0, n, tmp, 1, 1024);
  }
  return binv_build_rec(ctx, Lm->p, Lm->ld, 0, Linv, n, 0, n, tmp, 1);
}

int64_t chol_binv_order(int64_t n) { return potrs_block(n); }
int64_t chol_binv_elems(int64_t n) {
  const int64_t ib = potrs_block(n);
  return 2 * ((n + ib - 1) / ib) * ib * ib;
}

int chol_binv_finish(gpx_ctx* ctx, gpx_mat* Lm, int64_t ib) {
  const int64_t nblk = (Lm->prows + ib - 1) / ib, elems = nblk * ib * ib;
  dim3 gt((unsigned)(ib / 32), (unsigned)(ib / 32), (unsigned)nblk);
  hipLaunchKernelGGL(binv_transpose_kernel, gt, dim3(256), 0, ctx->stream, Lm->binv, Lm->binv + elems, ib);
  GPX_HIP(hipGetLastError());
  Lm->binv_ib = ib;
  return 0;
}

int chol_block_transpose(gpx_ctx* ctx, const double* in, double* out, int64_t n) {
  GPX_ARG(in && out && n > 0 && n % 32 == 0, "block transpose: order must be a multiple of 32");
  hipLaunchKernelGGL(binv_transpose_kernel, dim3((unsigned)(n / 32), (unsigned)(n / 32), 1), dim3(256), 0, ctx->stream, in, out, n);
  GPX_HIP(hipGetLastError());
  return 0;
}

int chol_tri_gemv(gpx_ctx* ctx, const double* M, int64_t ld, int64_t sz, const double* y, double* x, int lower) {
  GPX_ARG(M && y && x && x != y && sz > 0 && sz % NB == 0 && ld % 2 == 0, "triangular gemv: bad arguments");
  hipLaunchKernelGGL(binv_gemv_kernel, dim3((unsigned)((sz + 3) / 4)), dim3(256), 0, ctx->stream, M, ld, sz, y, x, lower);
  GPX_HIP(hipGetLastError());
  return 0;
}

int chol_binv_ensure(gpx_ctx* ctx, gpx_mat* Lm) {
  const int64_t n = Lm->prows, ib = potrs_block(n);
  if (Lm->binv && Lm->binv_ib == ib) return 0;
  const int64_t nblk = (n + ib - 1) / ib;
  const int64_t bytes = chol_binv_elems(n) * 8;
  if (Lm->binv && Lm->binv_bytes != bytes) {
    gpx_dev_release(ctx, Lm->binv, Lm->binv_bytes);
    Lm->binv = nullptr;
  }
  if (!Lm->binv) {
    void* p;
    GPX_TRY(gpx_dev_alloc(ctx, bytes, &p));
    Lm->binv = (double*)p;
    Lm->binv_bytes = bytes;
  }
  void* pt;
  GPX_TRY(gpx_dev_alloc(ctx, nblk * ib * ib * 8, &pt));
  int r = binv_build_range(ctx, Lm->p, Lm->ld, Lm->aux, Lm->binv, ib, n, (double*)pt);
  if (r == 0) r = chol_binv_finish(ctx, Lm, ib);
  (void)hipStreamSynchronize(ctx->stream);
  gpx_dev_release(ctx, pt, nblk * ib * ib * 8);
  if (r != 0) Lm->binv_ib = 0;
  return r;
}

struct PotrsPlan {
  const double* L;
  int64_t ld, n, ib, nblk;
  int64_t sib;
  const double* binv;
  const double* binvT;
  double* part;
  int strassen = 0;
  double* sscr = nullptr;
  int64_t sscr_bytes = 0;
};
static inline int64_t blk_off(const PotrsPlan& P, int64_t b) { return b * P.ib < P.n ? b * P.ib : P.n; }
static inline const double* blk_inv(const PotrsPlan& P, const double* base, int64_t b) {
  const int64_t row = b * P.ib, sb = row / P.sib, within = row - sb * P.sib;
  return base + sb * P.sib * P.sib + within * P.sib + within;
}

static int potrs_fwd(gpx_ctx* ctx, const PotrsPlan& P, int64_t b0, int64_t b1, double* rhs, double* x) {
  if (b1 - b0 == 1) {
    const int64_t o = blk_off(P, b0), sz = blk_off(P, b0 + 1) - o;
    hipLaunchKernelGGL(binv_gemv_kernel, dim3((unsigned)((sz + 3) / 4)), dim3(256), 0, ctx->stream, blk_inv(P, P.binv, b0),
                       P.sib, sz, rhs + o, x + o, 1);
    return 0;
  }
  const int64_t mid = (b0 + b1) / 2;
  GPX_TRY(potrs_fwd(ctx, P, b0, mid, rhs, x));
  const int64_t r0 = blk_off(P, mid), r1 = blk_off(P, b1), c0 = blk_off(P, b0);
  int64_t wg = (r1 - r0 + 3) / 4;
  if (wg > 4096) wg = 4096;
  hipLaunchKernelGGL(gemv_sub_kernel, dim3((unsigned)wg), dim3(256), 0, ctx->stream, P.L + r0 * P.ld + c0, P.ld, r1 - r0, r0 - c0,
                     x + c0, rhs + r0);
  return potrs_fwd(ctx, P, mid, b1, rhs, x);
}

static int potrs_bwd(gpx_ctx* ctx, const PotrsPlan& P, int64_t b0, int64_t b1, double* rhs, double* z) {
  if (b1 - b0 == 1) {
    const int64_t o = blk_off(P, b0), sz = blk_off(P, b0 + 1) - o;
    hipLaunchKernelGGL(binv_gemv_kernel, dim3((unsigned)((sz + 3) / 4)), dim3(256), 0, ctx->stream, blk_inv(P, P.binvT, b0),
                       P.sib, sz, rhs + o, z + o, 0);
    return 0;
  }
  const int64_t mid = (b0 + b1) / 2;
  GPX_TRY(potrs_bwd(ctx, P, mid, b1, rhs, z));
  const int64_t r0 = blk_off(P, mid), r1 = blk_off(P, b1), c0 = blk_off(P, b0);
  GPX_TRY(launch_colreduce(ctx, P.L + r0 * P.ld + c0, P.ld, r1 - r0, r0 - c0, z + r0, rhs + c0, P.part, 1));
  return potrs_bwd(ctx, P, b0, mid, rhs, z);
}

#ifndef GPX_STRASSEN_MIN_ROWS
#define GPX_STRASSEN_MIN_ROWS 8192
#endif
#ifndef GPX_STRASSEN_MIN_COLS
#define GPX_STRASSEN_MIN_COLS 4096
#endif
#ifndef GPX_STRASSEN2_MIN_ROWS
#define GPX_STRASSEN2_MIN_ROWS 16384
#endif
#ifndef GPX_STRASSEN2_MIN_COLS
#define GPX_STRASSEN2_MIN_COLS 16384
#endif
static inline int strassen_gate(int64_t rows, int64_t cols, int64_t k) {
  if (!(rows >= GPX_STRASSEN_MIN_ROWS && k >= GPX_STRASSEN_MIN_ROWS && cols >= GPX_STRASSEN_MIN_COLS &&
        gemm_strassen_scratch_bytes(rows, cols, k, 1) > 0))
    return 0;
  if (!(rows >= GPX_STRASSEN2_MIN_ROWS && k >= GPX_STRASSEN2_MIN_ROWS && cols >= GPX_STRASSEN2_MIN_COLS &&
        gemm_strassen_scratch_bytes(rows, cols, k, 2) > 0))
    return 1;
  return 2;
}

static int trsm_left_oop_rec(gpx_ctx* ctx, const PotrsPlan& P, int64_t b0, int64_t b1, double* B, int64_t ldb, double* W,
                             int64_t ldw, int64_t m) {
  if (b1 - b0 == 1) {
    const int64_t o = blk_off(P, b0), sz = blk_off(P, b0 + 1) - o;
    return launch_gemm_tri(ctx, blk_inv(P, P.binv, b0), P.sib, B + o * ldb, ldb, W + o * ldw, ldw, sz, m, sz, false, false,
                           false, 1);
  }
  const int64_t mid = (b0 + b1) / 2;
  GPX_TRY(trsm_left_oop_rec(ctx, P, b0, mid, B, ldb, W, ldw, m));
  const int64_t r0 = blk_off(P, mid), r1 = blk_off(P, b1), c0 = blk_off(P, b0);
  const int depth = P.strassen ? std::min(P.strassen, strassen_gate(r1 - r0, m, r0 - c0)) : 0;
  if (depth > 0)
    GPX_TRY(launch_gemm_strassen(ctx, P.L + r0 * P.ld + c0, P.ld, W + c0 * ldw, ldw, B + r0 * ldb, ldb, r1 - r0, m, r0 - c0,
                                 depth, P.sscr, P.sscr_bytes));
  else
    GPX_TRY(launch_gemm(ctx, P.L + r0 * P.ld + c0, P.ld, W + c0 * ldw, ldw, B + r0 * ldb, ldb, r1 - r0, m, r0 - c0, false,
                        true, false));
  return trsm_left_oop_rec(ctx, P, mid, b1, B, ldb, W, ldw, m);
}

int chol_trsm_left_oop(gpx_ctx* ctx, gpx_mat* Lm, double* B, int64_t ldb, double* W, int64_t ldw, int64_t m) {
  GPX_ARG(Lm && Lm->factored && Lm->aux && B && W && B != W, "trsm: matrix has not been factored / bad buffers");
  if (m == 0) return 0;
  GPX_TRY(chol_binv_ensure(ctx, Lm));
  PotrsPlan P;
  P.L = Lm->p;
  P.ld = Lm->ld;
  P.n = Lm->prows;
  P.sib = Lm->binv_ib;
  P.ib = P.sib < 1024 ? P.sib : 1024;
  P.nblk = (P.n + P.ib - 1) / P.ib;
  P.binv = Lm->binv;
  P.binvT = nullptr;
  P.part = nullptr;
  void* ps = nullptr;
  int64_t sbytes = 0;
  int depth = 0;
  const int64_t max_depth = env_i64("GPX_STRASSEN", GPX_STRASSEN_MAX_DEPTH);
  if (P.nblk >= 2 && max_depth > 0) {
    const int64_t r0 = blk_off(P, P.nblk / 2);
    for (depth = (int)std::min<int64_t>(max_depth, strassen_gate(P.n - r0, m, r0)); depth > 0; --depth) {
      sbytes = gemm_strassen_scratch_bytes(P.n - r0, m, r0, depth);
      if (sbytes > 0 && gpx_dev_alloc(ctx, sbytes, &ps) == 0) break;
      (void)hipGetLastError();
      ps = nullptr;
    }
  }
  P.strassen = ps ? depth : 0;
  P.sscr = (double*)ps;
  P.sscr_bytes = sbytes;
  const int r = trsm_left_oop_rec(ctx, P, 0, P.nblk, B, ldb, W, ldw, m);
  if (ps) {
    (void)hipStreamSynchronize(ctx->stream);
    gpx_dev_release(ctx, ps, sbytes);
  }
  return r;
}

int chol_trsm_left_group(gpx_ctx* ctx, const double* Lg, int64_t ld, const double* invd, int64_t w, int64_t below, int64_t ib,
                         double* B, int64_t ldb, int64_t m, double* inv, double* tmp, double* W, int64_t ldw) {
  GPX_ARG(Lg && invd && B && inv && tmp && W && W != B && w > 0 && w % NB == 0 && ib >= NB && ib % NB == 0, "trsm group: bad arguments");
  if (m == 0) return 0;
  GPX_TRY(binv_build_range(ctx, Lg, ld, invd, inv, ib, w, tmp));
  PotrsPlan P;
  P.L = Lg;
  P.ld = ld;
  P.n = w;
  P.ib = P.sib = ib;
  P.nblk = (w + ib - 1) / ib;
  P.binv = inv;
  P.binvT = nullptr;
  P.part = nullptr;
  GPX_TRY(trsm_left_oop_rec(ctx, P, 0, P.nblk, B, ldb, W, ldw, m));
  if (below > 0) GPX_TRY(launch_gemm(ctx, Lg + w * ld, ld, W, ldw, B + w * ldb, ldb, below, m, w, false, true, false));
  return gpx_copy2d(ctx, W, ldw, B, ldb, w, m);
}

int64_t chol_potrs_scratch_bytes(int64_t n) { return n * 8 + colreduce_partial_elems(n, n) * 8 + 64; }

int chol_potrs(gpx_ctx* ctx, gpx_mat* Lm, double* v, double* scratch) {
  GPX_ARG(Lm && Lm->factored && Lm->aux && v && scratch, "potrs: matrix has not been factored / NULL vector");
  GPX_ARG(Lm->ld % 2 == 0, "potrs: leading dimension must be even");
  GPX_TRY(chol_binv_ensure(ctx, Lm));
  PotrsPlan P;
  P.L = Lm->p;
  P.ld = Lm->ld;
  P.n = Lm->prows;
  P.ib = P.sib = Lm->binv_ib;
  P.nblk = (P.n + P.ib - 1) / P.ib;
  P.binv = Lm->binv;
  P.binvT = Lm->binv + P.nblk * P.ib * P.ib;
  P.part = scratch + P.n;
  double* x = scratch;
  ProfScope ps(ctx, GPX_PROF_TRSV, 2.0 * (double)P.n * P.n, 8.0 * (double)P.n * P.n);
  GPX_TRY(potrs_fwd(ctx, P, 0, P.nblk, v, x));
  GPX_TRY(potrs_bwd(ctx, P, 0, P.nblk, x, v));
  GPX_HIP(hipGetLastError());
  return 0;
}

int64_t chol_trsv_scratch_bytes(int64_t n) { return n * 8 + colreduce_partial_elems(n, n) * 8 + 64; }

int chol_trsv_with_scratch(gpx_ctx* ctx, const double* L, int64_t ld, const double* invd, double* y, int64_t n,
                           bool transposed, double* scratch) {
  GPX_ARG(n % NB == 0 && n > 0, "trsv: padded length must be a positive multiple of 128");
  GPX_ARG(ld % 2 == 0, "trsv: leading dimension must be even");
  ProfScope ps(ctx, GPX_PROF_TRSV, (double)n * n, 4.0 * (double)n * n);
  int r = transposed ? trsv_bwd_rec(ctx, L, ld, invd, y, n, scratch, scratch + n) : trsv_fwd_rec(ctx, L, ld, invd, y, n);
  if (r != 0) return r;
  GPX_HIP(hipGetLastError());
  return 0;
}

int chol_trsv(gpx_ctx* ctx, const double* L, int64_t ld, const double* invd, double* y, int64_t n, bool transposed) {
  if (!transposed) return chol_trsv_with_scratch(ctx, L, ld, invd, y, n, false, nullptr);
  void* p;
  const int64_t b = chol_trsv_scratch_bytes(n);
  GPX_TRY(gpx_dev_alloc(ctx, b, &p));
  int r = chol_trsv_with_scratch(ctx, L, ld, invd, y, n, true, (double*)p);
  (void)hipStreamSynchronize(ctx->stream);
  gpx_dev_release(ctx, p, b);
  return r;
}

int launch_gemv_sub(gpx_ctx* ctx, const double* A, int64_t ld, int64_t rows, int64_t cols, const double* x, double* y) {
  if (rows <= 0 || cols <= 0) return 0;
  GPX_ARG(cols % 2 == 0 && ld % 2 == 0, "gemv_sub: even column count and leading dimension");
  int64_t wg = (rows + 3) / 4;
  if (wg > 4096) wg = 4096;
  ProfScope ps(ctx, GPX_PROF_TRSV, 2.0 * (double)rows * cols, 8.0 * (double)rows * cols);
  hipLaunchKernelGGL(gemv_sub_kernel, dim3((unsigned)wg), dim3(256), 0, ctx->stream, A, ld, rows, cols, x, y);
  GPX_HIP(hipGetLastError());
  return 0;
}

int launch_logdet(gpx_ctx* ctx, const double* L, int64_t ld, int64_t n, double* d_out) {
  ProfScope ps(ctx, GPX_PROF_REDUCE, 0.0, 8.0 * (double)n);
  hipLaunchKernelGGL(logdet_kernel, dim3(1), dim3(256), 0, ctx->stream, L, ld, n, d_out);
  GPX_HIP(hipGetLastError());
  return 0;
}
```

gpexp_amd/csrc/gemm_f64.hip:

```cpp
#include "gpx_internal.h"
#include <stdlib.h>

namespace {

typedef double d4 __attribute__((ext_vector_type(4)));

constexpr int KB = 16;
constexpr int SA = KB + 1;

template <bool BT, int TE>
struct Smem {
  double a[2][TE * SA];
  double b[2][BT ? TE * SA : KB * (TE + 16)];
};

template <bool LOWER>
__device__ __forceinline__ bool tile_of(int sblk, int within, int tiles_m, int tiles_n, int sb_cols, int sb_shift,
                                        int* by, int* bx, int rot = 0) {
  const int sbm = (1 << sb_shift) - 1;
  int sr, sc;
  if (LOWER) {
    const int nsr = (tiles_m + sbm) >> sb_shift;
    const int noff = nsr * (nsr - 1) / 2;
    if (sblk < noff) {
// ... 721 lines not shown
  GPX_ARG(m % 128 == 0 && n % 128 == 0 && k % KB == 0 && k > 0 && m > 0 && n > 0, "gemm: m,n must be multiples of 128 and k of 16");
  GPX_ARG((lda % 2) == 0 && (ldb % 2) == 0, "gemm: leading dimensions must be even (16-byte loads)");
  const double tiles128 = (double)(m / 128) * (double)(n / 128);
  const int te = tiles128 < 1024.0 ? 64 : 128;
  const Plan p = make_plan(m, n, false, te);
  GPX_ARG(p.wgs < ((int64_t)1 << 31), "gemm: grid too large");
  const int nk = (int)(k / KB);
  ProfScope ps(ctx, GPX_PROF_GEMM, 2.0 * (double)m * (double)n * (double)k, 0.0);
  if (te == 64)
    hipLaunchKernelGGL(gemm_f64_dual_kernel<64>, dim3((unsigned)p.wgs), dim3(256), 0, ctx->stream, A, lda, B, ldb, C1, C2, s, ldc,
                       nk, p.tm, p.tn, p.sbc, p.sb_shift);
  else
    hipLaunchKernelGGL(gemm_f64_dual_kernel<128>, dim3((unsigned)p.wgs), dim3(256), 0, ctx->stream, A, lda, B, ldb, C1, C2, s, ldc,
                       nk, p.tm, p.tn, p.sbc, p.sb_shift);
  GPX_HIP(hipGetLastError());
  return 0;
}

static int launch_gemm_multi(gpx_ctx* ctx, const double* A, int64_t lda, const double* B, int64_t ldb, const Multi& dst,
                             int64_t ldc, int64_t m, int64_t n, int64_t k) {
  GPX_ARG(m % 128 == 0 && n % 128 == 0 && k % KB == 0 && k > 0 && m > 0 && n > 0, "gemm: m,n must be multiples of 128 and k of 16");
  GPX_ARG((lda % 2) == 0 && (ldb % 2) == 0, "gemm: leading dimensions must be even (16-byte loads)");
  GPX_ARG(dst.nd >= 1 && dst.nd <= GPX_MULTI_MAX, "gemm: bad destination count");
  const double tiles128 = (double)(m / 128) * (double)(n / 128);
  const int te = tiles128 < 1024.0 ? 64 : 128;
  const Plan p = make_plan(m, n, false, te);
  GPX_ARG(p.wgs < ((int64_t)1 << 31), "gemm: grid too large");
  const int nk = (int)(k / KB);
  ProfScope ps(ctx, GPX_PROF_GEMM, 2.0 * (double)m * (double)n * (double)k, 0.0);
  if (te == 64)
    hipLaunchKernelGGL(gemm_f64_multi_kernel<64>, dim3((unsigned)p.wgs), dim3(256), 0, ctx->stream, A, lda, B, ldb, dst, ldc, nk,
                       p.tm, p.tn, p.sbc, p.sb_shift);
  else
    hipLaunchKernelGGL(gemm_f64_multi_kernel<128>, dim3((unsigned)p.wgs), dim3(256), 0, ctx->stream, A, lda, B, ldb, dst, ldc, nk,
                       p.tm, p.tn, p.sbc, p.sb_shift);
  GPX_HIP(hipGetLastError());
  return 0;
}

static inline bool strassen_shape_ok(int64_t m, int64_t n, int64_t k, int depth) {
  return depth >= 1 && depth <= GPX_STRASSEN_MAX_DEPTH && m > 0 && n > 0 && k > 0 && m % ((int64_t)128 << depth) == 0 &&
         n % ((int64_t)128 << depth) == 0 && k % ((int64_t)KB << depth) == 0;
}

static inline int64_t strassen_level_elems(int64_t hm, int64_t hn, int64_t hk) {
  return 5 * (hm * gpx_skew_ld(hk) + hk * gpx_skew_ld(hn));
}

int64_t gemm_strassen_scratch_bytes(int64_t m, int64_t n, int64_t k, int depth) {
  if (!strassen_shape_ok(m, n, k, depth)) return 0;
  int64_t elems = 0;
  for (int d = 0; d < depth; ++d) {
    m /= 2, n /= 2, k /= 2;
    elems += strassen_level_elems(m, n, k);
  }
  return elems * 8;
}

namespace {
struct SDest {
  double* c;
  double s;
};
struct SProd {
  int a, b, nq, q[2];
  double s[2];
};
constexpr SProd kStrassen[7] = {
    {-1, -1, 2, {0, 3}, {1.0, 1.0}},
    {-2, 0, 2, {2, 3}, {1.0, -1.0}},
    {0, -2, 2, {1, 3}, {1.0, 1.0}},
    {3, -3, 2, {0, 2}, {1.0, 1.0}},
    {-3, 3, 2, {1, 0}, {1.0, -1.0}},
    {-4, -4, 1, {3, 0}, {1.0, 0.0}},
    {-5, -5, 1, {0, 0}, {1.0, 0.0}},
};
}

static int strassen_rec(gpx_ctx* ctx, const double* A, int64_t lda, const double* B, int64_t ldb, const SDest* dst, int nd,
                        int64_t ldc, int64_t m, int64_t n, int64_t k, int depth, double* scratch) {
  if (depth == 0) {
    for (int d = 1; d < nd; ++d)
      for (int e = 0; e < d; ++e) GPX_ARG(dst[d].c != dst[e].c, "strassen: two destinations of one product coincide");
    if (nd == 1 && dst[0].s == 1.0) return launch_gemm(ctx, A, lda, B, ldb, dst[0].c, ldc, m, n, k, false, true, false);
    if (nd == 2 && dst[0].s == 1.0) return launch_gemm_dual(ctx, A, lda, B, ldb, dst[0].c, dst[1].c, dst[1].s, ldc, m, n, k);
    GPX_ARG(nd >= 1 && nd <= GPX_MULTI_MAX, "strassen: too many destinations for one product");
    Multi md;
    for (int d = 0; d < GPX_MULTI_MAX; ++d) {
      md.c[d] = d < nd ? dst[d].c : nullptr;
      md.s[d] = d < nd ? dst[d].s : 0.0;
    }
    md.nd = nd;
    return launch_gemm_multi(ctx, A, lda, B, ldb, md, ldc, m, n, k);
  }
  const int64_t hm = m / 2, hn = n / 2, hk = k / 2, lsa = gpx_skew_ld(hk), lsb = gpx_skew_ld(hn);
  const int64_t sa = hm * lsa, sb = hk * lsb;
  double* const S = scratch;
  double* const T = scratch + 5 * sa;
  double* const below = T + 5 * sb;
  {
    ProfScope ps(ctx, GPX_PROF_REDUCE, 5.0 * (double)hm * hk + 5.0 * (double)hk * hn, 72.0 * ((double)hm * hk + (double)hk * hn));
    hipLaunchKernelGGL(strassen_sums_kernel<false>, dim3((unsigned)((hk / 2 + 255) / 256), (unsigned)(hm < 65535 ? hm : 65535)),
                       dim3(256), 0, ctx->stream, A, lda, hm, hk, S, lsa, sa);
    hipLaunchKernelGGL(strassen_sums_kernel<true>, dim3((unsigned)((hn / 2 + 255) / 256), (unsigned)(hk < 65535 ? hk : 65535)),
                       dim3(256), 0, ctx->stream, B, ldb, hk, hn, T, lsb, sb);
    if (hipGetLastError() != hipSuccess) {
      gpx_set_error("strassen: operand-sum launch failed");
      return -2;
    }
  }
  const int64_t qoff[4] = {0, hn, hm * ldc, hm * ldc + hn};
  for (const SProd& p : kStrassen) {
    const double* Ap = p.a < 0 ? S + (-1 - p.a) * sa : (p.a == 0 ? A : A + hm * lda + hk);
    const double* Bp = p.b < 0 ? T + (-1 - p.b) * sb : (p.b == 0 ? B : B + hk * ldb + hn);
    SDest sub[GPX_MULTI_MAX];
    int ns = 0;
    for (int d = 0; d < nd; ++d)
      for (int j = 0; j < p.nq; ++j) {
        GPX_ARG(ns < GPX_MULTI_MAX, "strassen: too many destinations for one product");
        sub[ns++] = SDest{dst[d].c + qoff[p.q[j]], dst[d].s * p.s[j]};
      }
    GPX_TRY(strassen_rec(ctx, Ap, p.a < 0 ? lsa : lda, Bp, p.b < 0 ? lsb : ldb, sub, ns, ldc, hm, hn, hk, depth - 1, below));
  }
  return 0;
}

int launch_gemm_strassen(gpx_ctx* ctx, const double* A, int64_t lda, const double* B, int64_t ldb, double* C, int64_t ldc,
                         int64_t m, int64_t n, int64_t k, int depth, double* scratch, int64_t scratch_bytes) {
  if (depth > GPX_STRASSEN_MAX_DEPTH) depth = GPX_STRASSEN_MAX_DEPTH;
  if ((lda % 2) != 0 || (ldb % 2) != 0 || C == A || C == B) depth = 0;
  void* own = nullptr;
  int64_t need = 0;
  for (; depth > 0; --depth) {
    need = gemm_strassen_scratch_bytes(m, n, k, depth);
    if (need == 0) continue;
    if (scratch && scratch_bytes >= need) break;
    if (gpx_dev_alloc(ctx, need, &own) == 0) {
      scratch = (double*)own;
      break;
    }
    (void)hipGetLastError();
    own = nullptr;
  }
  if (depth <= 0) return launch_gemm(ctx, A, lda, B, ldb, C, ldc, m, n, k, false, true, false);
  const SDest top{C, 1.0};
  const int r = strassen_rec(ctx, A, lda, B, ldb, &top, 1, ldc, m, n, k, depth, scratch);
  if (own) {
    (void)hipStreamSynchronize(ctx->stream);
    gpx_dev_release(ctx, own, need);
  }
  return r;
}

int launch_dist2_update(gpx_ctx* ctx, double* C, int64_t ldc, int64_t lr0, int64_t m, int64_t lc0, int64_t n, int64_t nb, int Pr,
                        int Pc, int pr, int pc, int64_t piece_stride, int64_t dsz, int nseg, const double* const* g,
                        const int64_t* ks, int below_diag) {
  if (m == 0 || n == 0 || nseg == 0) return 0;
  GPX_ARG(nseg > 0 && nseg <= GPX_SEG_MAX && Pr >= 1 && Pr <= GPX_MAX_PR && Pc >= 1, "dist2 update: too many segments / grid rows");
  GPX_ARG(m % 128 == 0 && n % 128 == 0 && nb % 128 == 0 && lr0 % nb == 0 && lc0 % nb == 0 && (ldc % 2) == 0, "dist2 update: alignment");
  Dist2Upd u;
  for (int s = 0; s < nseg; ++s) {
    u.g[s] = g[s];
    for (int p = 0; p < Pr; ++p) u.li0[s][p] = (int)(ks[s] + 1 <= p ? 0 : (ks[s] - p) / Pr + 1);
  }
  u.nseg = nseg;
  u.seg_nk = (int)(nb / KB);
  u.Pr = Pr; u.Pc = Pc; u.pr = pr; u.pc = pc;
  u.nb = (int)nb;
  u.gld = (int)gpx_g_ld(nb);
  u.li_first = (int)(lr0 / nb);
  u.lj_first = (int)(lc0 / nb);
  u.below_diag = below_diag;
  u.piece_stride = piece_stride;
  u.dsz = dsz;
  double tiles128 = 0.0;
  for (int64_t lj = lc0 / nb; lj * nb < lc0 + n; ++lj) {
    const int64_t J = lj * Pc + pc;
    const int64_t cw = (lc0 + n - lj * nb) < nb ? (lc0 + n - lj * nb) : nb;
    for (int64_t li = lr0 / nb; li * nb < lr0 + m; ++li) {
      const int64_t I = li * Pr + pr;
      if (I < J || (below_diag && I == J)) continue;
      const int64_t rh = (lr0 + m - li * nb) < nb ? (lr0 + m - li * nb) : nb;
      tiles128 += (double)(rh / 128) * (double)(cw / 128);
    }
  }
  if (tiles128 == 0.0) return 0;
  constexpr int small_max = 512;
  const int te = tiles128 < (double)small_max ? 64 : 128;
  const int tm = (int)(m / te), tn = (int)(n / te), tpb = (int)(nb / te);
  u.nsc = (tn + 7) / 8;
  u.nsr = (tm + 7) / 8;
  GPX_ARG(u.nsc <= GPX_SC_MAX, "dist2 update: too many column super-blocks in one launch");
  int64_t nfull = 0, npart = 0;
  for (int sc = 0; sc < u.nsc; ++sc) {
    const int64_t lj = lc0 / nb + (8 * sc) / tpb, J = lj * Pc + pc;
    int64_t li_min = (J + (below_diag ? 1 : 0) - pr + Pr - 1) / Pr;
    if (J + (below_diag ? 1 : 0) - pr < 0) li_min = 0;
    int64_t by_min = (li_min - lr0 / nb) * tpb;
    if (by_min < 0) by_min = 0;
    int srm = (int)(by_min / 8);
    if (srm > u.nsr) srm = u.nsr;
    u.sr_min[sc] = srm;
    int64_t bx_right = 8 * (int64_t)sc + 7;
    if (bx_right > tn - 1) bx_right = tn - 1;
    const int64_t ljr = lc0 / nb + bx_right / tpb, Jr = ljr * Pc + pc;
    int64_t li_full = (Jr + (below_diag ? 1 : 0) - pr + Pr - 1) / Pr;
    if (Jr + (below_diag ? 1 : 0) - pr < 0) li_full = 0;
    int64_t by_full = (li_full - lr0 / nb) * tpb;
    if (by_full < 0) by_full = 0;
    int srf = (int)((by_full + 7) / 8);
    if (srf < srm) srf = srm;
    if (srf > u.nsr) srf = u.nsr;
    u.sr_full[sc] = srf;
    u.prefix_p[sc] = (int)npart;
    u.prefix_f[sc] = (int)nfull;
    npart += srf - srm;
    nfull += u.nsr - srf;
  }
  u.prefix_p[u.nsc] = (int)npart;
  u.prefix_f[u.nsc] = (int)nfull;
  u.nfull = (int)nfull;
  const int64_t nsb = nfull + npart;
  if (nsb == 0) return 0;
  const int64_t wgs = (nsb + 7) / 8 * 8 * 64;
  GPX_ARG(wgs < ((int64_t)1 << 31), "dist2 update: grid too large");
  ProfScope ps(ctx, GPX_PROF_GEMM, 2.0 * tiles128 * 128.0 * 128.0 * (double)nb * nseg, 0.0);
  double* Cb = C + lr0 * ldc + lc0;
  if (te == 64)
    hipLaunchKernelGGL(dist2_update_kernel<64>, dim3((unsigned)wgs), dim3(256), 0, ctx->stream, u, Cb, ldc, tm, tn);
  else
    hipLaunchKernelGGL(dist2_update_kernel<128>, dim3((unsigned)wgs), dim3(256), 0, ctx->stream, u, Cb, ldc, tm, tn);
  GPX_HIP(hipGetLastError());
  return 0;
}
```

gpexp_amd/csrc/gpx_internal.h:

```cpp
#pragma once
#include <hip/hip_runtime.h>
#include <stdint.h>
#include <stdlib.h>
#include <string>
#include <vector>
#include <map>
#include <memory>
#include <unordered_set>
#include "../../include/gpx.h"
#include "../../include/gpx_dist.h"
#include "../../include/gpx_debug.h"

#define GPX_TILE 128
#define GPX_MAXD GPX_MAX_DIM
#define GPX_NSTREAMS 6
#define GPX_SEG_MAX 8
#ifndef GPX_G_SKEW
#define GPX_G_SKEW 0
#endif
#define GPX_MAX_PR 4

void gpx_set_error(const char* fmt, ...);
#define GPX_HIP(call)                                                                   \
  do {                                                                                  \
    hipError_t e_ = (call);                                                             \
    if (e_ != hipSuccess) {                                                             \
      gpx_set_error("%s:%d %s -> %s", __FILE__, __LINE__, #call, hipGetErrorString(e_)); \
      return -2;                                                                        \
    }                                                                                   \
  } while (0)
#define GPX_ARG(cond, msg)                                   \
  do {                                                       \
    if (!(cond)) {                                           \
      gpx_set_error("%s:%d bad argument: %s", __FILE__, __LINE__, msg); \
      return -1;                                             \
    }                                                        \
  } while (0)
#define GPX_TRY(call)        \
  do {                       \
    int r_ = (call);         \
    if (r_ != 0) return r_;  \
  } while (0)

static inline int64_t gpx_round_up(int64_t v, int64_t m) { return (v + m - 1) / m * m; }
static inline int64_t gpx_skew_ld(int64_t cols) { return (cols >= 1024 && cols % 256 == 0) ? cols + 16 : cols; }

static inline int64_t gpx_g_ld(int64_t nb) { return nb + GPX_G_SKEW; }

struct KParams {
  int kind;
  int d;
  double sig;
  double scale[GPX_MAXD];
  double c1[GPX_MAXD];
  double c2[GPX_MAXD];
  double center[GPX_MAXD];
  int exact;
};
int gpx_make_kparams(int kind, int d, const double* hyp, int nhyp, KParams* out);

static __device__ __forceinline__ double kpair(const KParams& kp, const double* __restrict__ a, const double* __restrict__ b) {
  double acc = 0.0;
  if (kp.kind == GPX_K_MEHLER) {
    double pa = 0.0, pb = 0.0, cr = 0.0;
    for (int k = 0; k < kp.d; ++k) {
      const double x = a[k], y = b[k];
      pa = fma(kp.c1[k] * x, x, pa);
      pb = fma(kp.c1[k] * y, y, pb);
      cr = fma(kp.c2[k] * x, y, cr);
    }
    return kp.sig * exp(-(pa + pb - cr));
  }
  for (int k = 0; k < kp.d; ++k) {
    const double e = (a[k] - b[k]) * kp.scale[k];
    acc = fma(e, e, acc);
  }
  if (kp.kind == GPX_K_SE) return kp.sig * exp(-0.5 * acc);
  const double t = sqrt(acc);
  if (kp.kind == GPX_K_MATERN32) return kp.sig * (1.0 + t) * exp(-t);
  return kp.sig * (1.0 + t + acc * (1.0 / 3.0)) * exp(-t);
}

struct gpx_mat {
  double* p;
  int64_t rows, cols;
  int64_t prows, pcols;
  int64_t ld;
  int64_t bytes;
  double* aux;
  int64_t aux_bytes;
  int factored;
  int bbox_ok;
  double lo[GPX_MAXD], hi[GPX_MAXD];
  int64_t bad_row, bad_col;
  double* binv;
  int64_t binv_bytes;
  int64_t binv_ib;
  double* dinv;
  int64_t dinv_bytes;
  int64_t dinv_nb;
  std::vector<unsigned char> dinv_ok;
};

struct ProfRec {
  hipEvent_t a, b;
  int cls;
  hipStream_t stream;
  bool open;
};

struct gpx_ctx {
  int device;
  hipStream_t stream;
  hipStream_t streams[GPX_NSTREAMS];
  std::vector<hipEvent_t> sync_events;
  std::unordered_set<const gpx_mat*> live_mats;
  double* pw_binv;
  int64_t pw_ib;
  double* pw_tmp_build;
  double* pw_tmp_T;
  int pw_done;
  std::vector<hipEvent_t> la_events;
  hipEvent_t ev_side = nullptr;
  int cus;
  std::multimap<int64_t, void*> pool;
  int64_t pool_bytes;
  struct Fence {
    std::vector<hipEvent_t> evs;
  };
  std::map<void*, std::shared_ptr<Fence>> pending;
  std::vector<hipEvent_t> fence_free;
  int guard;
  int64_t guard_violations;
  uint64_t chaos;
  int* d_info;
  double piv_min;
  int piv_skip;
  double* d_scal;
  double* trsv_scratch;
  int64_t trsv_scratch_bytes;
  double* d2_scratch;
  int64_t d2_scratch_bytes;
  long long* dbg_stamps;
  const double* d2_inv_src;
  int64_t d2_inv_nb;
  double* ev_scratch;
  int64_t ev_scratch_bytes;
  void* comm;
  int rank, world;
  void* grp[3];
  int grp_size[3], grp_rank[3];
  int Pr, Pc;
  int prof_on;
  std::vector<ProfRec> prof_recs;
  std::vector<hipEvent_t> ev_free;
  int64_t prof_launches[GPX_PROF_NCLASS];
  double prof_ms[GPX_PROF_NCLASS];
  double prof_flops[GPX_PROF_NCLASS];
  double prof_bytes[GPX_PROF_NCLASS];
};

int gpx_kparams_sets(gpx_ctx* ctx, KParams* kp, const gpx_mat* A, const gpx_mat* B = nullptr, const gpx_mat* C = nullptr);
int gpx_dev_alloc(gpx_ctx* ctx, int64_t bytes, void** out);
void gpx_dev_release(gpx_ctx* ctx, void* p, int64_t bytes);
int gpx_mat_new(gpx_ctx* ctx, int64_t rows, int64_t cols, int pad, gpx_mat** out);

struct ProfScope {
  gpx_ctx* ctx;
  int idx;
  ProfScope(gpx_ctx* c, int cls, double flops, double bytes);
  ~ProfScope();
};
int gpx_prof_flush(gpx_ctx* ctx);

#define GPX_SE_DISPATCH(d_, CALL) \
  do {                            \
    if ((d_) <= 1) { CALL(1); }   \
    else if ((d_) <= 2) { CALL(2); } \
    else if ((d_) <= 4) { CALL(4); } \
    else if ((d_) <= 8) { CALL(8); } \
    else if ((d_) <= 16) { CALL(16); } \
    else { CALL(32); }            \
  } while (0)

extern "C" int64_t gpx_eval_chunk(int64_t np);

int launch_kfill(gpx_ctx* ctx, const KParams& kp, const double* A, int64_t na, const double* B, int64_t nb,
                 int symmetric, const double* d_nugget, int64_t nugget_len, double nugget_scalar,
                 double* out, int64_t prows, int64_t pcols, int64_t ld);
int launch_kfill_offset(gpx_ctx* ctx, const KParams& kp, const double* X, int64_t n, int64_t row_off, int64_t col_off,
                        const double* d_nugget, int64_t nugget_len, double nugget_scalar, double* out, int64_t prows,
                        int64_t pcols, int64_t ld);
int launch_kdiag(gpx_ctx* ctx, const KParams& kp, const double* Z, int64_t m, double* out);
int launch_kfill_cyclic(gpx_ctx* ctx, const KParams& kp, const double* X, int64_t n, const double* d_nugget,
                        int64_t nugget_len, double nugget_scalar, double* out, int64_t prows, int64_t pcols, int64_t ld,
                        int64_t nb, int Pr, int pr, int Pc, int pc);
int gpx_copy2d(gpx_ctx* ctx, const double* src, int64_t lds_, double* dst, int64_t ldd, int64_t rows, int64_t cols);
int gpx_copy2d_lower(gpx_ctx* ctx, const double* src, int64_t lds_, double* dst, int64_t ldd, int64_t n);
int launch_kfill_rows(gpx_ctx* ctx, const KParams& kp, const double* X, int64_t n, int64_t row0, const double* d_nugget,
                      int64_t nugget_len, double nugget_scalar, double* out, int64_t prows_band, int64_t pcols,
                      int64_t ld);

static inline int gpx_chain_prio(const gpx_ctx* ctx) { return ctx->stream == ctx->streams[1] ? 1 : 0; }
int launch_gemm(gpx_ctx* ctx, const double* A, int64_t lda, const double* B, int64_t ldb, double* C, int64_t ldc,
                int64_t m, int64_t n, int64_t k, bool bt, bool accumulate, bool lower);

int launch_gemm_tri(gpx_ctx* ctx, const double* A, int64_t lda, const double* B, int64_t ldb, double* C, int64_t ldc,
                    int64_t m, int64_t n, int64_t k, bool bt, bool accumulate, bool lower, int tri);
constexpr int GPX_STRASSEN_MAX_DEPTH = 2;
int64_t gemm_strassen_scratch_bytes(int64_t m, int64_t n, int64_t k, int depth);
int launch_gemm_strassen(gpx_ctx* ctx, const double* A, int64_t lda, const double* B, int64_t ldb, double* C, int64_t ldc,
                         int64_t m, int64_t n, int64_t k, int depth, double* scratch, int64_t scratch_bytes);
int launch_gemm_ksplit(gpx_ctx* ctx, const double* A, int64_t lda, const double* B, int64_t ldb, double* C, int64_t ldc,
                       int64_t m, int64_t n, int64_t k, bool lower, int64_t parts, double* P, bool assign = false);
int launch_gemm_ksplit_small(gpx_ctx* ctx, const double* A, int64_t lda, const double* B, int64_t ldb, double* C, int64_t ldc,
                             int64_t m, int64_t n, int64_t k, bool assign, int64_t parts, double* P);
int launch_gemm_batched(gpx_ctx* ctx, const double* A, int64_t lda, int64_t sa, const double* B, int64_t ldb, int64_t sb,
                        double* C, int64_t ldc, int64_t sc, int64_t m, int64_t n, int64_t k, bool bt, bool accumulate,
                        int64_t batch);

int launch_dist2_update(gpx_ctx* ctx, double* C, int64_t ldc, int64_t lr0, int64_t m, int64_t lc0, int64_t n, int64_t nb, int Pr,
                        int Pc, int pr, int pc, int64_t piece_stride, int64_t dsz, int nseg, const double* const* g,
                        const int64_t* ks, int below_diag);

int launch_leaf(gpx_ctx* ctx, double* A, int64_t ld, double* inv, int64_t base_index, int64_t n_valid);
int chol_potrf(gpx_ctx* ctx, double* A, int64_t ld, int64_t n, double* invd, int64_t n_valid);
int chol_potrf_nozero(gpx_ctx* ctx, double* A, int64_t ld, int64_t n, double* invd, int64_t base, int64_t n_valid);
int chol_trsm_right(gpx_ctx* ctx, const double* L, int64_t ldl, const double* invd, double* X, int64_t ldx,
                    int64_t m, int64_t n);
int chol_trsm_right_n(gpx_ctx* ctx, const double* L, int64_t ldl, const double* invd, double* X, int64_t ldx,
                      int64_t m, int64_t n);
int chol_trsm_left(gpx_ctx* ctx, const double* L, int64_t ldl, const double* invd, double* B, int64_t ldb,
                   int64_t n, int64_t m);
int chol_trsv(gpx_ctx* ctx, const double* L, int64_t ld, const double* invd, double* y, int64_t n, bool transposed);
int64_t chol_trsv_scratch_bytes(int64_t n);
int chol_trsv_with_scratch(gpx_ctx* ctx, const double* L, int64_t ld, const double* invd, double* y, int64_t n,
                           bool transposed, double* scratch);
int launch_logdet(gpx_ctx* ctx, const double* L, int64_t ld, int64_t n, double* d_out);
int chol_trtri(gpx_ctx* ctx, const gpx_mat* L, double* Linv, double* tmp);
int chol_binv_ensure(gpx_ctx* ctx, gpx_mat* L);
int chol_trsm_right_trailing(gpx_ctx* ctx, gpx_mat* L, int64_t r0, double* X, int64_t ldx, int64_t m, int transposed, double* T);
int chol_trsm_right_leading(gpx_ctx* ctx, gpx_mat* L, int64_t ncols, double* X, int64_t ldx, int64_t m, double* T, int64_t tcap);
int chol_trsm_right_n_leading(gpx_ctx* ctx, gpx_mat* L, int64_t ncols, double* X, int64_t ldx, int64_t m, double* T);
int chol_block_inverse(gpx_ctx* ctx, const double* D, int64_t ldd, const double* invd, double* inv, int64_t w, double* tmp);
int64_t chol_binv_order(int64_t n);
int64_t chol_binv_elems(int64_t n);
int chol_binv_finish(gpx_ctx* ctx, gpx_mat* L, int64_t ib);
int chol_trsm_left_oop(gpx_ctx* ctx, gpx_mat* L, double* B, int64_t ldb, double* W, int64_t ldw, int64_t m);
int chol_trsm_left_group(gpx_ctx* ctx, const double* Lg, int64_t ld, const double* invd, int64_t w, int64_t below, int64_t ib,
                         double* B, int64_t ldb, int64_t m, double* inv, double* tmp, double* W, int64_t ldw);
int64_t chol_potrf_panel_width(int64_t n);
int64_t chol_potrs_scratch_bytes(int64_t n);
int chol_potrs(gpx_ctx* ctx, gpx_mat* L, double* v, double* scratch);
int launch_gemv_sub(gpx_ctx* ctx, const double* A, int64_t ld, int64_t rows, int64_t cols, const double* x, double* y);
int chol_block_transpose(gpx_ctx* ctx, const double* in, double* out, int64_t n);
int chol_tri_gemv(gpx_ctx* ctx, const double* M, int64_t ld, int64_t sz, const double* y, double* x, int lower);

struct gpx_fitc;
int64_t fitc_n(const gpx_fitc* f);
int64_t fitc_np(const gpx_fitc* f);
int64_t fitc_nup(const gpx_fitc* f);
int fitc_solve_beta_t(gpx_ctx* ctx, const gpx_fitc* f, const double* B, int64_t mcp, double* Bt, double* U);

int launch_colreduce(gpx_ctx* ctx, const double* B, int64_t ld, int64_t rows, int64_t pcols, const double* v,
                     double* out, double* d_partial, int subtract = 0);
int64_t colreduce_partial_elems(int64_t rows, int64_t pcols);
int launch_rowreduce(gpx_ctx* ctx, const double* B, int64_t ld, int64_t rows, int64_t cols, const double* v,
                     double* out, int weighted_squares = 0);
int launch_sum(gpx_ctx* ctx, const double* x, int64_t n, double* d_out);

extern "C" int gpx_potri_impl(gpx_ctx* ctx, const gpx_mat* L, gpx_mat** outP, int full);
int launch_transpose(gpx_ctx* ctx, const double* in, int64_t rows, int64_t cols, int64_t ldi, double* out, int64_t ldo);
```

gpexp_amd/csrc/reduce.hip:

```cpp
#include "gpx_internal.h"

namespace {

constexpr int ROWS_PER_CHUNK_MIN = 16;

__global__ __launch_bounds__(256) void colreduce_kernel(const double* __restrict__ B, int64_t ld, int64_t rows,
                                                        int64_t chunk, const double* __restrict__ v,
                                                        double* __restrict__ partial, int64_t pcols) {
  const int64_t j = (int64_t)blockIdx.x * 256 + threadIdx.x;
  const int64_t r0 = (int64_t)blockIdx.y * chunk;
  int64_t r1 = r0 + chunk;
  if (r1 > rows) r1 = rows;
  if (j >= pcols) return;
  double s0 = 0.0, s1 = 0.0, s2 = 0.0, s3 = 0.0;
  const double* p = B + r0 * ld + j;
  int64_t i = r0;
  if (v) {
    for (; i + 4 <= r1; i += 4, p += 4 * ld) {
      s0 = fma(p[0], v[i], s0);
      s1 = fma(p[ld], v[i + 1], s1);
      s2 = fma(p[2 * ld], v[i + 2], s2);
      s3 = fma(p[3 * ld], v[i + 3], s3);
    }
    for (; i < r1; ++i, p += ld) s0 = fma(p[0], v[i], s0);
  } else {
    for (; i + 4 <= r1; i += 4, p += 4 * ld) {
      double a = p[0], b = p[ld], c = p[2 * ld], d = p[3 * ld];
      s0 = fma(a, a, s0);
      s1 = fma(b, b, s1);
      s2 = fma(c, c, s2);
      s3 = fma(d, d, s3);
    }
    for (; i < r1; ++i, p += ld) s0 = fma(p[0], p[0], s0);
  }
  partial[(int64_t)blockIdx.y * pcols + j] = (s0 + s1) + (s2 + s3);
}

__global__ __launch_bounds__(256) void colreduce_final_kernel(const double* __restrict__ partial, int64_t nchunk,
                                                              int64_t pcols, double* __restrict__ out, int subtract) {
  const int64_t j = (int64_t)blockIdx.x * 256 + threadIdx.x;
  if (j >= pcols) return;
  double s0 = 0.0, s1 = 0.0, s2 = 0.0, s3 = 0.0;
  const double* p = partial + j;
  int64_t c = 0;
  for (; c + 4 <= nchunk; c += 4, p += 4 * pcols) {
    const double a = p[0], b = p[pcols], d = p[2 * pcols], e = p[3 * pcols];
    s0 += a;
    s1 += b;
    s2 += d;
    s3 += e;
  }
  for (; c < nchunk; ++c, p += pcols) s0 += p[0];
  const double s = (s0 + s1) + (s2 + s3);
  out[j] = subtract ? out[j] - s : s;
}

__global__ __launch_bounds__(256) void sum_kernel(const double* __restrict__ x, int64_t n, double* __restrict__ out) {
  __shared__ double red[256];
  double s = 0.0;
  for (int64_t i = threadIdx.x; i < n; i += 256) s += x[i];
  red[threadIdx.x] = s;
  __syncthreads();
  for (int w = 128; w > 0; w >>= 1) {
    if (threadIdx.x < w) red[threadIdx.x] += red[threadIdx.x + w];
    __syncthreads();
  }
  if (threadIdx.x == 0) out[0] = red[0];
}

inline void plan(int64_t rows, int64_t pcols, int64_t* chunk, int64_t* nchunk) {
  int64_t colblocks = (pcols + 255) / 256;
  int64_t want = 2048 / colblocks;
  if (want < 1) want = 1;
  int64_t maxc = (rows + ROWS_PER_CHUNK_MIN - 1) / ROWS_PER_CHUNK_MIN;
  if (maxc < 1) maxc = 1;
  if (want > maxc) want = maxc;
  *chunk = (rows + want - 1) / want;
  if (*chunk < 1) *chunk = 1;
  *nchunk = (rows + *chunk - 1) / *chunk;
  if (*nchunk < 1) *nchunk = 1;
}

}

int64_t colreduce_partial_elems(int64_t rows, int64_t pcols) {
  const int64_t by_rows = ((rows + ROWS_PER_CHUNK_MIN - 1) / ROWS_PER_CHUNK_MIN + 1) * pcols;
  const int64_t cap = (int64_t)2048 * 256 + pcols;
  return by_rows < cap ? by_rows : cap;
}

int launch_colreduce(gpx_ctx* ctx, const double* B, int64_t ld, int64_t rows, int64_t pcols, const double* v,
                     double* out, double* d_partial, int subtract) {
  int64_t chunk, nchunk;
  plan(rows, pcols, &chunk, &nchunk);
  GPX_ARG(nchunk * pcols <= colreduce_partial_elems(rows, pcols), "colreduce: partial-sum plan exceeds its own bound");
  ProfScope ps(ctx, GPX_PROF_REDUCE, 2.0 * (double)rows * pcols, 8.0 * (double)rows * pcols);
  dim3 grid((unsigned)((pcols + 255) / 256), (unsigned)nchunk);
  hipLaunchKernelGGL(colreduce_kernel, grid, dim3(256), 0, ctx->stream, B, ld, rows, chunk, v, d_partial, pcols);
  hipLaunchKernelGGL(colreduce_final_kernel, dim3(grid.x), dim3(256), 0, ctx->stream, d_partial, nchunk, pcols, out,
                     subtract);
  GPX_HIP(hipGetLastError());
  return 0;
}

namespace {

__global__ __launch_bounds__(256) void rowreduce_kernel(const double* __restrict__ B, int64_t ld, int64_t cols,
                                                        const double* __restrict__ v, double* __restrict__ out,
                                                        int weighted_squares) {
  __shared__ double red[256];
  const int t = threadIdx.x;
  const double* row = B + (int64_t)blockIdx.x * ld;
  double s0 = 0.0, s1 = 0.0;
  if (v && weighted_squares) {
    for (int64_t c = 2 * t; c < cols; c += 512) {
      const double2 b = *reinterpret_cast<const double2*>(row + c);
      const double2 w = *reinterpret_cast<const double2*>(v + c);
      s0 = fma(b.x * w.x, b.x, s0);
      s1 = fma(b.y * w.y, b.y, s1);
    }
  } else if (v) {
    for (int64_t c = 2 * t; c < cols; c += 512) {
      const double2 b = *reinterpret_cast<const double2*>(row + c);
      const double2 w = *reinterpret_cast<const double2*>(v + c);
      s0 = fma(b.x, w.x, s0);
      s1 = fma(b.y, w.y, s1);
    }
  } else {
    for (int64_t c = 2 * t; c < cols; c += 512) {
      const double2 b = *reinterpret_cast<const double2*>(row + c);
      s0 = fma(b.x, b.x, s0);
      s1 = fma(b.y, b.y, s1);
    }
  }
  red[t] = s0 + s1;
  __syncthreads();
  for (int w = 128; w > 0; w >>= 1) {
    if (t < w) red[t] += red[t + w];
    __syncthreads();
  }
  if (t == 0) out[blockIdx.x] = red[0];
}

}

int launch_rowreduce(gpx_ctx* ctx, const double* B, int64_t ld, int64_t rows, int64_t cols, const double* v,
                     double* out, int weighted_squares) {
  if (rows <= 0) return 0;
  GPX_ARG(cols % 2 == 0 && ld % 2 == 0, "rowreduce: even column count and leading dimension");
  ProfScope ps(ctx, GPX_PROF_REDUCE, 2.0 * (double)rows * cols, 8.0 * (double)rows * cols);
  hipLaunchKernelGGL(rowreduce_kernel, dim3((unsigned)rows), dim3(256), 0, ctx->stream, B, ld, cols, v, out,
                     weighted_squares);
  GPX_HIP(hipGetLastError());
  return 0;
}

int launch_sum(gpx_ctx* ctx, const double* x, int64_t n, double* d_out) {
  hipLaunchKernelGGL(sum_kernel, dim3(1), dim3(256), 0, ctx->stream, x, n, d_out);
  GPX_HIP(hipGetLastError());
  return 0;
}

extern "C" int gpx_dbg_colreduce_plan(int64_t rows, int64_t pcols, int64_t* nchunk, int64_t* bound_elems) {
  if (rows < 1 || pcols < 1 || !nchunk || !bound_elems) return -1;
  int64_t chunk;
  plan(rows, pcols, &chunk, nchunk);
  *bound_elems = colreduce_partial_elems(rows, pcols);
  return 0;
}
```

gpexp_amd/device.py:

```python
import ctypes as C
import atexit
import os

import numpy as np

from . import _lib
from ._lib import check, as_f64, dptr, c_vp, c_i64, GpxError

K_SE, K_MATERN32, K_MATERN52, K_MEHLER = 0, 1, 2, 3
PROF_CLASSES = ["kfill", "gemm", "leaf", "trsv", "reduce", "greedy", "comm", "kcross"]

_ctx = None


class Context:

    def __init__(self, device=None):
        self.lib = _lib.load()
        if device is None:
            device = int(os.environ.get("LOCAL_RANK", "0"))
        h = c_vp()
        rc = self.lib.gpx_create(int(device), C.byref(h))
        if rc != 0:
            raise RuntimeError("gpexp_amd needs an MI355X: " + self.lib.gpx_last_error().decode())
# ... 539 lines not shown
        self.h = h

    def row(self, cur, rowbuf):
        check(self.ctx.lib.gpx_mi_row(self.ctx.h, self.h, int(cur), int(self.picks[cur]), rowbuf.h))

    def score(self, cur, rowbuf):
        v = C.c_double()
        i = c_i64()
        check(self.ctx.lib.gpx_mi_score(self.ctx.h, self.h, int(cur), rowbuf.h, C.byref(v), C.byref(i)))
        return v.value, i.value

    def select(self, slot, idx):
        check(self.ctx.lib.gpx_mi_select(self.ctx.h, self.h, int(slot), int(idx)))
        assert slot == len(self.picks)
        self.picks.append(int(idx))

    def __del__(self):
        try:
            if self.h and self.ctx.h:
                self.ctx.lib.gpx_mi_end(self.ctx.h, self.h)
            self.h = None
        except Exception:
            pass


def alloc_vector(ctx, n):
    return DeviceMatrix.zeros(ctx, max(int(n), 1), 1, pad=False)


def lml_grad_slab_bounds(n, parts):
    npad = (max(n, 1) + 127) // 128 * 128
    q = 1024 if npad >= 8192 else 128
    b = [int(round(npad * (1.0 - (1.0 - i / parts) ** (1.0 / 3.0)) / q)) * q for i in range(parts + 1)]
    b[0], b[-1] = 0, npad
    for i in range(1, parts + 1):
        b[i] = max(b[i], b[i - 1])
    return b


def lml_grad_slab(ctx, spec, L, X, alpha, r0, r1):
    alpha = as_f64(alpha)
    out = np.empty(spec.nsums)
    check(ctx.lib.gpx_lml_grad_slab(ctx.h, *spec.args(), L.h, X.h, dptr(alpha), int(r0), int(r1), dptr(out)))
    return out


def lml_grad_rows_bounds(n, parts, nsub=1):
    npad = (max(n, 1) + 127) // 128 * 128
    nsub = max(1, int(nsub))

    def cost(a, b):
        h = (b - a) / nsub
        return sum(h * (a + (j + 1) * h) ** 2 for j in range(nsub))

    def layout(t):
        b = [0.0]
        for _ in range(parts):
            lo, hi = b[-1], float(npad)
            if cost(b[-1], hi) <= t:
                b.append(hi)
                continue
            for _ in range(60):
                mid = 0.5 * (lo + hi)
                if cost(b[-1], mid) < t:
                    lo = mid
                else:
                    hi = mid
            b.append(hi)
        return b

    lo, hi = 0.0, cost(0.0, float(npad))
    for _ in range(60):
        t = 0.5 * (lo + hi)
        if layout(t)[-1] >= npad - 1e-6:
            hi = t
        else:
            lo = t
    b = [int(round(v / 128)) * 128 for v in layout(hi)]
    b[0], b[-1] = 0, npad
    for i in range(1, parts + 1):
        b[i] = min(max(b[i], b[i - 1]), npad)
    return b


def lml_grad_rows(ctx, spec, L, X, alpha, r0, r1, nsub=1):
    alpha = as_f64(alpha)
    out = np.empty(spec.nsums)
    check(ctx.lib.gpx_lml_grad_rows(ctx.h, *spec.args(), L.h, X.h, dptr(alpha), int(r0), int(r1), int(nsub), dptr(out)))
    return out


def lml_grad_from_sums(spec, sums):
    d = spec.nlen
    g = np.empty(d + 2)
    g[:d] = 0.5 * sums[:d] / spec.hyp[:d]
    g[d] = 0.5 * sums[d] / spec.hyp[d]
    g[d + 1] = 0.5 * sums[d + 1]
    return g


def ivar_grad(ctx, spec, L, X, Z, noise_deriv=None, W=None):
    out = np.empty(X.shape[0] * spec.d)
    nd = as_f64(noise_deriv) if noise_deriv is not None else None
    check(ctx.lib.gpx_ivar_grad_w(ctx.h, *spec.args(), L.h, X.h, Z.h, dptr(nd), W.h if W is not None else None, dptr(out)))
    return out


def ivar_grad_rows(ctx, spec, L, X, Z, W, r0):
    out = np.empty((X.shape[0] - int(r0)) * spec.d)
    check(ctx.lib.gpx_ivar_grad_rows(ctx.h, *spec.args(), L.h, X.h, Z.h, W.h, int(r0), dptr(out)))
    return out


def var_grad(ctx, spec, L, X, Z, noise_deriv=None, eval_bias=None, dk_bias=None):
    out = np.empty((X.shape[0] * spec.d, Z.shape[0]))
    nd = as_f64(noise_deriv) if noise_deriv is not None else None
    eb = as_f64(eval_bias) if eval_bias is not None else None
    db = as_f64(dk_bias) if dk_bias is not None else None
    check(ctx.lib.gpx_var_grad(ctx.h, *spec.args(), L.h, X.h, Z.h, dptr(nd), dptr(eb), dptr(db), dptr(out)))
    return out


def var_grad_newpt(ctx, spec, L, X, Z):
    out = np.empty(Z.shape[0] * spec.d)
    check(ctx.lib.gpx_var_grad_newpt(ctx.h, *spec.args(), L.h, X.h, Z.h, dptr(out)))
    return out


def kfill_plan(ctx, spec, X, Z=None):
    ex = C.c_int()
    cen = np.zeros(spec.d)
    check(ctx.lib.gpx_dbg_kfill_plan(ctx.h, *spec.args(), X.h, Z.h if Z is not None else None, C.byref(ex), dptr(cen)))
    return bool(ex.value), cen


def dbg_gemm_tri(ctx, A, B, Cm, bt, accumulate, tri):
    check(ctx.lib.gpx_dbg_gemm_tri(ctx.h, A.h, B.h, Cm.h, int(bt), int(accumulate), int(tri)))


def dbg_gemm_ksplit(ctx, A, B, Cm, mode, parts):
    check(ctx.lib.gpx_dbg_gemm_ksplit(ctx.h, A.h, B.h, Cm.h, int(mode), int(parts)))


def dbg_gemm(ctx, A, B, Cm, bt, accumulate, lower=False):
    check(ctx.lib.gpx_dbg_gemm(ctx.h, A.h, B.h, Cm.h, int(bt), int(accumulate), int(lower)))


def dbg_gemm_strassen(ctx, A, B, Cm):
    check(ctx.lib.gpx_dbg_gemm_strassen(ctx.h, A.h, B.h, Cm.h))


def dbg_gemm_strassen_depth(ctx, A, B, Cm, depth):
    check(ctx.lib.gpx_dbg_gemm_strassen_depth(ctx.h, A.h, B.h, Cm.h, int(depth)))
```

include/gpx_debug.h:

```cpp
#ifndef GPX_DEBUG_H
#define GPX_DEBUG_H
#include "gpx.h"
#ifdef __cplusplus
extern "C" {
#endif

int gpx_dbg_gemm(gpx_ctx* ctx, const gpx_mat* A, const gpx_mat* B, gpx_mat* C, int bt, int accumulate, int lower);
int gpx_dbg_gemm_tri(gpx_ctx* ctx, const gpx_mat* A, const gpx_mat* B, gpx_mat* C, int bt, int accumulate, int tri);
int gpx_dbg_gemm_ksplit(gpx_ctx* ctx, const gpx_mat* A, const gpx_mat* B, gpx_mat* C, int mode, int parts);
int gpx_dbg_gemm_strassen(gpx_ctx* ctx, const gpx_mat* A, const gpx_mat* B, gpx_mat* C);
int gpx_dbg_gemm_strassen_depth(gpx_ctx* ctx, const gpx_mat* A, const gpx_mat* B, gpx_mat* C, int depth);
int gpx_dbg_spin(gpx_ctx* ctx, int ms);
int64_t gpx_dbg_guard_violations(gpx_ctx* ctx);
int gpx_dbg_guard_selftest(gpx_ctx* ctx);
int gpx_dbg_panel_bcast_plan(int W, int me, int64_t small_elems, int npieces, const int64_t* counts, const int* roots,
                             int64_t* ops, int64_t max_ops, int64_t* nops);
int gpx_dbg_colreduce_plan(int64_t rows, int64_t pcols, int64_t* nchunk, int64_t* bound_elems);
int gpx_dbg_kfill_plan(gpx_ctx* ctx, int kind, int d, const double* hyp, int nhyp, const gpx_mat* X, const gpx_mat* Z,
                       int* exact, double* center);

int gpx_dbg_spin_us(gpx_ctx* ctx, int64_t us);
int gpx_dbg_stamp(gpx_ctx* ctx, int slot);
int gpx_dbg_spin_until(gpx_ctx* ctx, int slot, int64_t us);
int gpx_dbg_event_elapsed(gpx_ctx* ctx, int id0, int id1, double* ms);

int gpx_dbg_leaf_stamps(gpx_ctx* ctx, gpx_mat* K, int fast, int64_t* out30);

#ifdef __cplusplus
}
#endif
#endif
```

Measured before the change: 105,200 points/s.

## Overlap Strassen operand sums and column reductions with triangular solve on side stream

```diff
diff --git a/gpexp_amd/_lib.py b/gpexp_amd/_lib.py
--- a/gpexp_amd/_lib.py
+++ b/gpexp_amd/_lib.py
@@ -157,6 +157,7 @@
     "gpx_dbg_gemm": (C.c_int, [c_vp, c_vp, c_vp, c_vp, C.c_int, C.c_int, C.c_int]),
     "gpx_dbg_gemm_strassen": (C.c_int, [c_vp, c_vp, c_vp, c_vp]),
     "gpx_dbg_gemm_strassen_depth": (C.c_int, [c_vp, c_vp, c_vp, c_vp, C.c_int]),
+    "gpx_dbg_trsm_left_oop": (C.c_int, [c_vp, c_vp, c_vp, c_vp, C.POINTER(c_i64), C.POINTER(c_i64), c_i64, c_i64, c_dp]),
     "gpx_dbg_gemm_tri": (C.c_int, [c_vp, c_vp, c_vp, c_vp, C.c_int, C.c_int, C.c_int]),
     "gpx_dbg_gemm_ksplit": (C.c_int, [c_vp, c_vp, c_vp, c_vp, C.c_int, C.c_int]),
     "gpx_dbg_kfill_plan": (C.c_int, [c_vp, C.c_int, C.c_int, c_dp, C.c_int, c_vp, c_vp, C.POINTER(C.c_int), c_dp]),
diff --git a/gpexp_amd/csrc/api.hip b/gpexp_amd/csrc/api.hip
--- a/gpexp_amd/csrc/api.hip
+++ b/gpexp_amd/csrc/api.hip
@@ -165,6 +165,29 @@
   return 0;
 }
 
+hipEvent_t gpx_ov_event(gpx_ctx* ctx) {
+  if (ctx->ov_next == ctx->ov_events.size()) {
+    hipEvent_t ev;
+    if (hipEventCreateWithFlags(&ev, hipEventDisableTiming) != hipSuccess) {
+      (void)hipGetLastError();
+      return nullptr;
+    }
+    ctx->ov_events.push_back(ev);
+  }
+  return ctx->ov_events[ctx->ov_next++];
+}
+
+int gpx_ov_fork(gpx_ctx* ctx, hipStream_t from, hipStream_t to) {
+  hipEvent_t ev = gpx_ov_event(ctx);
+  if (!ev) {
+    gpx_set_error("solve overlap: no event to be had");
+    return -2;
+  }
+  GPX_HIP(hipEventRecord(ev, from));
+  GPX_HIP(hipStreamWaitEvent(to, ev, 0));
+  return 0;
+}
+
 int gpx_make_kparams(int kind, int d, const double* hyp, int nhyp, KParams* kp) {
   GPX_ARG(d >= 1 && d <= GPX_MAXD, "dimension must be in [1, GPX_MAX_DIM]");
   GPX_ARG(hyp != nullptr, "hyp is NULL");
@@ -508,6 +531,7 @@
   for (auto ev : ctx->sync_events) (void)hipEventDestroy(ev);
   for (auto ev : ctx->la_events) (void)hipEventDestroy(ev);
   if (ctx->ev_side) (void)hipEventDestroy(ctx->ev_side);
+  for (auto ev : ctx->ov_events) (void)hipEventDestroy(ev);
   for (int i = 0; i < GPX_NSTREAMS; ++i) {
     bool seen = false;
     for (int j = 0; j < i; ++j) seen = seen || ctx->streams[j] == ctx->streams[i];
@@ -1180,13 +1204,16 @@
       }
       if (var) {
         const double* Wsol = B;
+        TrsmColsums cs{n, (double*)ppart, 0};
         if (oop) {
-          if ((r = chol_trsm_left_oop(ctx, const_cast<gpx_mat*>(L), B, ldb, (double*)pW, ldb, mcp)) != 0) break;
+          if ((r = chol_trsm_left_oop(ctx, const_cast<gpx_mat*>(L), B, ldb, (double*)pW, ldb, mcp, &cs)) != 0) break;
           Wsol = (const double*)pW;
         } else if ((r = chol_trsm_left(ctx, L->p, L->ld, L->aux, B, ldb, np, mcp)) != 0) {
           break;
         }
-        if ((r = launch_colreduce(ctx, Wsol, ldb, n, mcp, nullptr, (double*)pout, (double*)ppart)) != 0) break;
+        if (cs.done) r = launch_colreduce_final(ctx, (const double*)ppart, n, mcp, (double*)pout);
+        else r = launch_colreduce(ctx, Wsol, ldb, n, mcp, nullptr, (double*)pout, (double*)ppart);
+        if (r != 0) break;
         if ((r = launch_kdiag(ctx, kp, Zc, mc, (double*)pkd)) != 0) break;
         hipLaunchKernelGGL(vec_diff_kernel, dim3((unsigned)((mc + 255) / 256)), dim3(256), 0, ctx->stream, (const double*)pkd,
                            (const double*)pout, mc, var_dev + j0);
@@ -1472,4 +1499,38 @@
   return 0;
 }
 
-}
+int gpx_dbg_trsm_left_oop(gpx_ctx* ctx, gpx_mat* L, gpx_mat* B, gpx_mat* W, const int64_t* min_rows, const int64_t* min_cols,
+                          int64_t scratch_cap, int64_t sum_rows, double* colsums) {
+  GPX_ARG(ctx && L && B && W && min_rows && min_cols, "NULL argument");
+  GPX_TRY(need_factor(L));
+  const int64_t np = L->prows, mcp = B->pcols;
+  GPX_ARG(B->prows == np && W->prows == np && W->pcols == mcp && mcp % GPX_TILE == 0 && np % GPX_TILE == 0, "trsm hook: shapes");
+  GPX_ARG(colsums == nullptr || (sum_rows > 0 && sum_rows <= np), "trsm hook: rows of the column sums");
+  const TrsmTune tune{{min_rows[0], min_rows[1]}, {min_cols[0], min_cols[1]}, scratch_cap};
+  void *pout = nullptr, *ppart = nullptr;
+  const int64_t bytes_out = mcp * 8, bytes_part = colsums ? colreduce_partial_elems(sum_rows, mcp) * 8 + 8 : 0;
+  int r = 0;
+  do {
+    TrsmColsums cs{sum_rows, nullptr, 0};
+    if (colsums) {
+      if ((r = gpx_dev_alloc(ctx, bytes_out, &pout)) != 0) break;
+      if ((r = gpx_dev_alloc(ctx, bytes_part, &ppart)) != 0) break;
+      cs.partial = (double*)ppart;
+    }
+    if ((r = chol_trsm_left_oop(ctx, L, B->p, B->ld, W->p, W->ld, mcp, colsums ? &cs : nullptr, &tune)) != 0) break;
+    if (colsums) {
+      if (cs.done) r = launch_colreduce_final(ctx, (const double*)ppart, sum_rows, mcp, (double*)pout);
+      else r = launch_colreduce(ctx, W->p, W->ld, sum_rows, mcp, nullptr, (double*)pout, (double*)ppart);
+      if (r == 0 && hipMemcpyAsync(colsums, pout, (size_t)mcp * 8, hipMemcpyDeviceToHost, ctx->stream) != hipSuccess) {
+        gpx_set_error("trsm hook: copy of the column sums failed");
+        r = -2;
+      }
+    }
+  } while (0);
+  (void)hipStreamSynchronize(ctx->stream);
+  if (pout) gpx_dev_release(ctx, pout, bytes_out);
+  if (ppart) gpx_dev_release(ctx, ppart, bytes_part);
+  return r;
+}
+
+}
diff --git a/gpexp_amd/csrc/chol.hip b/gpexp_amd/csrc/chol.hip
--- a/gpexp_amd/csrc/chol.hip
+++ b/gpexp_amd/csrc/chol.hip
@@ -1226,6 +1226,8 @@
   int strassen = 0;
   double* sscr = nullptr;
   int64_t sscr_bytes = 0;
+  const int64_t* gates = nullptr;
+  struct SolveOverlap* ov = nullptr;
 };
 static inline int64_t blk_off(const PotrsPlan& P, int64_t b) { return b * P.ib < P.n ? b * P.ib : P.n; }
 static inline const double* blk_inv(const PotrsPlan& P, const double* base, int64_t b) {
@@ -1276,28 +1278,78 @@
 #ifndef GPX_STRASSEN2_MIN_COLS
 #define GPX_STRASSEN2_MIN_COLS 16384
 #endif
-static inline int strassen_gate(int64_t rows, int64_t cols, int64_t k) {
-  if (!(rows >= GPX_STRASSEN_MIN_ROWS && k >= GPX_STRASSEN_MIN_ROWS && cols >= GPX_STRASSEN_MIN_COLS &&
-        gemm_strassen_scratch_bytes(rows, cols, k, 1) > 0))
-    return 0;
-  if (!(rows >= GPX_STRASSEN2_MIN_ROWS && k >= GPX_STRASSEN2_MIN_ROWS && cols >= GPX_STRASSEN2_MIN_COLS &&
-        gemm_strassen_scratch_bytes(rows, cols, k, 2) > 0))
-    return 1;
+static const int64_t kStrassenGates[4] = {GPX_STRASSEN_MIN_ROWS, GPX_STRASSEN_MIN_COLS, GPX_STRASSEN2_MIN_ROWS,
+                                          GPX_STRASSEN2_MIN_COLS};
+static inline int strassen_gate(int64_t rows, int64_t cols, int64_t k, const int64_t* g = nullptr) {
+  if (!g) g = kStrassenGates;
+  if (!(rows >= g[0] && k >= g[0] && cols >= g[1] && gemm_strassen_scratch_bytes(rows, cols, k, 1) > 0)) return 0;
+  if (!(rows >= g[2] && k >= g[2] && cols >= g[3] && gemm_strassen_scratch_bytes(rows, cols, k, 2) > 0)) return 1;
   return 2;
+}
+
+struct AheadUpd {
+  int64_t r0, r1, c0;
+  int depth;
+  double* S;
+  hipEvent_t ready;
+};
+struct SolveOverlap {
+  hipStream_t main, side;
+  bool sums = false;
+  std::vector<AheadUpd> upd;
+  size_t next_upd = 0;
+  double* T = nullptr;
+  TrsmColsums* cs = nullptr;
+  int64_t chunk = 0, nchunk = 0, next_chunk = 0;
+  bool side_used = false;
+};
+
+static void collect_updates(const PotrsPlan& P, int64_t b0, int64_t b1, int64_t m, int cap, std::vector<AheadUpd>& out) {
+  if (b1 - b0 == 1) return;
+  const int64_t mid = (b0 + b1) / 2;
+  collect_updates(P, b0, mid, m, cap, out);
+  const int64_t r0 = blk_off(P, mid), r1 = blk_off(P, b1), c0 = blk_off(P, b0);
+  const int depth = std::min(cap, strassen_gate(r1 - r0, m, r0 - c0, P.gates));
+  if (depth > 0) out.push_back(AheadUpd{r0, r1, c0, depth, nullptr, nullptr});
+  collect_updates(P, mid, b1, m, cap, out);
+}
+
+static int colsums_advance(gpx_ctx* ctx, SolveOverlap& ov, const double* W, int64_t ldw, int64_t m, int64_t done) {
+  const int64_t rows = ov.cs->rows;
+  const int64_t c1 = done >= rows ? ov.nchunk : done / ov.chunk;
+  if (c1 <= ov.next_chunk) return 0;
+  GPX_TRY(gpx_ov_fork(ctx, ov.main, ov.side));
+  ov.side_used = true;
+  ctx->stream = ov.side;
+  const int r = launch_colreduce_chunks(ctx, W, ldw, rows, m, ov.next_chunk, c1, ov.cs->partial);
+  ctx->stream = ov.main;
+  ov.next_chunk = c1;
+  return r;
 }
 
 static int trsm_left_oop_rec(gpx_ctx* ctx, const PotrsPlan& P, int64_t b0, int64_t b1, double* B, int64_t ldb, double* W,
                              int64_t ldw, int64_t m) {
   if (b1 - b0 == 1) {
     const int64_t o = blk_off(P, b0), sz = blk_off(P, b0 + 1) - o;
-    return launch_gemm_tri(ctx, blk_inv(P, P.binv, b0), P.sib, B + o * ldb, ldb, W + o * ldw, ldw, sz, m, sz, false, false,
-                           false, 1);
+    GPX_TRY(launch_gemm_tri(ctx, blk_inv(P, P.binv, b0), P.sib, B + o * ldb, ldb, W + o * ldw, ldw, sz, m, sz, false, false,
+                            false, 1));
+    if (P.ov && P.ov->cs) GPX_TRY(colsums_advance(ctx, *P.ov, W, ldw, m, o + sz));
+    return 0;
   }
   const int64_t mid = (b0 + b1) / 2;
   GPX_TRY(trsm_left_oop_rec(ctx, P, b0, mid, B, ldb, W, ldw, m));
   const int64_t r0 = blk_off(P, mid), r1 = blk_off(P, b1), c0 = blk_off(P, b0);
-  const int depth = P.strassen ? std::min(P.strassen, strassen_gate(r1 - r0, m, r0 - c0)) : 0;
-  if (depth > 0)
+  const int depth = P.strassen ? std::min(P.strassen, strassen_gate(r1 - r0, m, r0 - c0, P.gates)) : 0;
+  if (depth > 0 && P.ov && P.ov->sums) {
+    SolveOverlap& ov = *P.ov;
+    GPX_ARG(ov.next_upd < ov.upd.size(), "trsm: more gated updates than were planned");
+    const AheadUpd& u = ov.upd[ov.next_upd++];
+    GPX_ARG(u.r0 == r0 && u.r1 == r1 && u.c0 == c0 && u.depth == depth, "trsm: the sweep and its plan of gated updates disagree");
+    GPX_HIP(hipStreamWaitEvent(ov.main, u.ready, 0));
+    if (depth > 1) ov.side_used = true;
+    GPX_TRY(launch_gemm_strassen_ahead(ctx, P.L + r0 * P.ld + c0, P.ld, W + c0 * ldw, ldw, B + r0 * ldb, ldb, r1 - r0, m, r0 - c0,
+                                       depth, u.S, ov.T, ov.side));
+  } else if (depth > 0)
     GPX_TRY(launch_gemm_strassen(ctx, P.L + r0 * P.ld + c0, P.ld, W + c0 * ldw, ldw, B + r0 * ldb, ldb, r1 - r0, m, r0 - c0,
                                  depth, P.sscr, P.sscr_bytes));
   else
@@ -1306,8 +1358,10 @@
   return trsm_left_oop_rec(ctx, P, mid, b1, B, ldb, W, ldw, m);
 }
 
-int chol_trsm_left_oop(gpx_ctx* ctx, gpx_mat* Lm, double* B, int64_t ldb, double* W, int64_t ldw, int64_t m) {
+int chol_trsm_left_oop(gpx_ctx* ctx, gpx_mat* Lm, double* B, int64_t ldb, double* W, int64_t ldw, int64_t m,
+                       TrsmColsums* colsums, const TrsmTune* tune) {
   GPX_ARG(Lm && Lm->factored && Lm->aux && B && W && B != W, "trsm: matrix has not been factored / bad buffers");
+  if (colsums) colsums->done = 0;
   if (m == 0) return 0;
   GPX_TRY(chol_binv_ensure(ctx, Lm));
   PotrsPlan P;
@@ -1320,23 +1374,89 @@
   P.binv = Lm->binv;
   P.binvT = nullptr;
   P.part = nullptr;
+  int64_t gates[4];
+  if (tune) {
+    gates[0] = tune->min_rows[0], gates[1] = tune->min_cols[0], gates[2] = tune->min_rows[1], gates[3] = tune->min_cols[1];
+    P.gates = gates;
+  }
+  const int64_t cap = tune ? tune->scratch_cap : -1;
+  const int64_t mask = env_i64("GPX_SOLVE_OVERLAP", GPX_OVERLAP_ALL);
+  SolveOverlap ov;
+  ov.main = ctx->stream;
+  ov.side = ctx->streams[4];
+  const bool can = ov.main == ctx->streams[0] && ov.side != ov.main;
+  const bool want_sums = can && (mask & GPX_OVERLAP_SUMS);
+  if (can && (mask & GPX_OVERLAP_COLSUMS) && colsums && colsums->partial && colsums->rows > 0 && colsums->rows <= P.n) {
+    ov.cs = colsums;
+    colreduce_plan(colsums->rows, m, &ov.chunk, &ov.nchunk);
+  }
   void* ps = nullptr;
   int64_t sbytes = 0;
   int depth = 0;
   const int64_t max_depth = env_i64("GPX_STRASSEN", GPX_STRASSEN_MAX_DEPTH);
   if (P.nblk >= 2 && max_depth > 0) {
     const int64_t r0 = blk_off(P, P.nblk / 2);
-    for (depth = (int)std::min<int64_t>(max_depth, strassen_gate(P.n - r0, m, r0)); depth > 0; --depth) {
+    for (depth = (int)std::min<int64_t>(max_depth, strassen_gate(P.n - r0, m, r0, P.gates)); depth > 0; --depth) {
+      if (want_sums) {
+        ov.upd.clear();
+        collect_updates(P, 0, P.nblk, m, depth, ov.upd);
+        int64_t lbytes = 0, rbytes = 0;
+        for (const AheadUpd& u : ov.upd) {
+          lbytes += gemm_strassen_left_bytes(u.r1 - u.r0, u.r0 - u.c0, u.depth);
+          rbytes = std::max(rbytes, gemm_strassen_right_bytes(m, u.r0 - u.c0, u.depth));
+        }
+        sbytes = lbytes + rbytes;
+        if (!ov.upd.empty() && (cap < 0 || sbytes <= cap) && gpx_dev_alloc(ctx, sbytes, &ps) == 0) {
+          double* q = (double*)ps;
+          for (AheadUpd& u : ov.upd) {
+            u.S = q;
+            q += gemm_strassen_left_bytes(u.r1 - u.r0, u.r0 - u.c0, u.depth) / 8;
+          }
+          ov.T = q;
+          ov.sums = true;
+          break;
+        }
+        (void)hipGetLastError();
+        ps = nullptr;
+      }
       sbytes = gemm_strassen_scratch_bytes(P.n - r0, m, r0, depth);
-      if (sbytes > 0 && gpx_dev_alloc(ctx, sbytes, &ps) == 0) break;
+      if (sbytes > 0 && (cap < 0 || sbytes <= cap) && gpx_dev_alloc(ctx, sbytes, &ps) == 0) break;
       (void)hipGetLastError();
       ps = nullptr;
     }
   }
   P.strassen = ps ? depth : 0;
-  P.sscr = (double*)ps;
-  P.sscr_bytes = sbytes;
-  const int r = trsm_left_oop_rec(ctx, P, 0, P.nblk, B, ldb, W, ldw, m);
+  P.sscr = ov.sums ? nullptr : (double*)ps;
+  P.sscr_bytes = ov.sums ? 0 : sbytes;
+  int r = 0;
+  if (ov.sums || ov.cs) {
+    P.ov = &ov;
+    ctx->ov_next = 0;
+  }
+  if (ov.sums) {
+    r = gpx_ov_fork(ctx, ov.main, ov.side);
+    ov.side_used = true;
+    ctx->stream = ov.side;
+    for (size_t i = 0; i < ov.upd.size() && r == 0; ++i) {
+      AheadUpd& u = ov.upd[i];
+      r = launch_strassen_left_sums(ctx, P.L + u.r0 * P.ld + u.c0, P.ld, u.r1 - u.r0, u.r0 - u.c0, u.depth, u.S);
+      if (r == 0 && (!(u.ready = gpx_ov_event(ctx)) || hipEventRecord(u.ready, ov.side) != hipSuccess)) {
+        gpx_set_error("trsm: no event for the operand sums");
+        r = -2;
+      }
+    }
+    ctx->stream = ov.main;
+  }
+  if (r == 0) r = trsm_left_oop_rec(ctx, P, 0, P.nblk, B, ldb, W, ldw, m);
+  if (ov.side_used) {
+    if (r == 0) r = gpx_ov_fork(ctx, ov.side, ov.main);
+    if (r != 0) (void)hipStreamSynchronize(ov.side);
+    (void)hipStreamSynchronize(ov.main);
+  }
+  if (r == 0 && ov.cs) {
+    if (ov.next_chunk == ov.nchunk) colsums->done = 1;
+    else { gpx_set_error("trsm: column sums incomplete"); r = -1; }
+  }
   if (ps) {
     (void)hipStreamSynchronize(ctx->stream);
     gpx_dev_release(ctx, ps, sbytes);
diff --git a/gpexp_amd/csrc/gemm_f64.hip b/gpexp_amd/csrc/gemm_f64.hip
--- a/gpexp_amd/csrc/gemm_f64.hip
+++ b/gpexp_amd/csrc/gemm_f64.hip
@@ -897,6 +897,103 @@
   return r;
 }
 
+int64_t gemm_strassen_left_bytes(int64_t m, int64_t k, int depth) {
+  if (depth < 1 || depth > GPX_STRASSEN_MAX_DEPTH) return 0;
+  int64_t elems = 5 * (m / 2) * gpx_skew_ld(k / 2);
+  if (depth == 2) elems += 7 * 5 * (m / 4) * gpx_skew_ld(k / 4);
+  return elems * 8;
+}
+
+int64_t gemm_strassen_right_bytes(int64_t n, int64_t k, int depth) {
+  if (depth < 1 || depth > GPX_STRASSEN_MAX_DEPTH) return 0;
+  int64_t elems = 5 * (k / 2) * gpx_skew_ld(n / 2);
+  if (depth == 2) elems += 2 * 5 * (k / 4) * gpx_skew_ld(n / 4);
+  return elems * 8;
+}
+
+static int launch_sums(gpx_ctx* ctx, bool bside, const double* X, int64_t ldx, int64_t hr, int64_t hc, double* S, int64_t lds) {
+  ProfScope ps(ctx, GPX_PROF_REDUCE, 5.0 * (double)hr * hc, 72.0 * (double)hr * hc);
+  const dim3 grid((unsigned)((hc / 2 + 255) / 256), (unsigned)(hr < 65535 ? hr : 65535));
+  if (bside)
+    hipLaunchKernelGGL(strassen_sums_kernel<true>, grid, dim3(256), 0, ctx->stream, X, ldx, hr, hc, S, lds, hr * lds);
+  else
+    hipLaunchKernelGGL(strassen_sums_kernel<false>, grid, dim3(256), 0, ctx->stream, X, ldx, hr, hc, S, lds, hr * lds);
+  if (hipGetLastError() != hipSuccess) {
+    gpx_set_error("strassen: operand-sum launch failed");
+    return -2;
+  }
+  return 0;
+}
+
+int launch_strassen_left_sums(gpx_ctx* ctx, const double* A, int64_t lda, int64_t m, int64_t k, int depth, double* S) {
+  GPX_ARG(depth >= 1 && depth <= GPX_STRASSEN_MAX_DEPTH && (lda % 2) == 0, "strassen: bad depth / odd leading dimension");
+  const int64_t hm = m / 2, hk = k / 2, lsa = gpx_skew_ld(hk), sa = hm * lsa;
+  GPX_TRY(launch_sums(ctx, false, A, lda, hm, hk, S, lsa));
+  if (depth < 2) return 0;
+  const int64_t qm = hm / 2, qk = hk / 2, lqa = gpx_skew_ld(qk), sqa = qm * lqa;
+  double* Sin = S + 5 * sa;
+  for (int p = 0; p < 7; ++p) {
+    const SProd& pr = kStrassen[p];
+    const double* Ap = pr.a < 0 ? S + (-1 - pr.a) * sa : (pr.a == 0 ? A : A + hm * lda + hk);
+    GPX_TRY(launch_sums(ctx, false, Ap, pr.a < 0 ? lsa : lda, qm, qk, Sin + p * 5 * sqa, lqa));
+  }
+  return 0;
+}
+
+int launch_gemm_strassen_ahead(gpx_ctx* ctx, const double* A, int64_t lda, const double* B, int64_t ldb, double* C, int64_t ldc,
+                               int64_t m, int64_t n, int64_t k, int depth, const double* S, double* T, hipStream_t side) {
+  GPX_ARG(strassen_shape_ok(m, n, k, depth) && (lda % 2) == 0 && (ldb % 2) == 0 && C != A && C != B && S && T,
+          "strassen: shape / operands the scheme refuses");
+  const hipStream_t main = ctx->stream;
+  const int64_t hm = m / 2, hn = n / 2, hk = k / 2, lsa = gpx_skew_ld(hk), lsb = gpx_skew_ld(hn);
+  const int64_t sa = hm * lsa, sb = hk * lsb;
+  const int64_t qm = hm / 2, qn = hn / 2, qk = hk / 2, lqa = gpx_skew_ld(qk), lqb = gpx_skew_ld(qn);
+  const int64_t sqa = qm * lqa, sqb = qk * lqb;
+  const double* Sin = S + 5 * sa;
+  double* Tin[2] = {T + 5 * sb, T + 5 * sb + 5 * sqb};
+  GPX_TRY(launch_sums(ctx, true, B, ldb, hk, hn, T, lsb));
+  const int64_t qoff[4] = {0, hn, hm * ldc, hm * ldc + hn}, qoff2[4] = {0, qn, qm * ldc, qm * ldc + qn};
+  auto opA = [&](int p) { const SProd& pr = kStrassen[p]; return pr.a < 0 ? S + (-1 - pr.a) * sa : (pr.a == 0 ? A : A + hm * lda + hk); };
+  auto opB = [&](int p) { const SProd& pr = kStrassen[p]; return pr.b < 0 ? T + (-1 - pr.b) * sb : (pr.b == 0 ? B : B + hk * ldb + hn); };
+  if (depth == 2) {
+    GPX_TRY(launch_sums(ctx, true, opB(0), kStrassen[0].b < 0 ? lsb : ldb, qk, qn, Tin[0], lqb));
+  }
+  for (int p = 0; p < 7; ++p) {
+    const SProd& pr = kStrassen[p];
+    const double* Ap = opA(p);
+    const double* Bp = opB(p);
+    const int64_t lap = pr.a < 0 ? lsa : lda, lbp = pr.b < 0 ? lsb : ldb;
+    SDest sub[GPX_MULTI_MAX];
+    int ns = 0;
+    for (int j = 0; j < pr.nq; ++j) sub[ns++] = SDest{C + qoff[pr.q[j]], pr.s[j]};
+    if (depth == 1) {
+      GPX_TRY(strassen_rec(ctx, Ap, lap, Bp, lbp, sub, ns, ldc, hm, hn, hk, 0, nullptr));
+      continue;
+    }
+    if (p + 1 < 7) {
+      GPX_TRY(gpx_ov_fork(ctx, main, side));
+      ctx->stream = side;
+      int r = launch_sums(ctx, true, opB(p + 1), kStrassen[p + 1].b < 0 ? lsb : ldb, qk, qn, Tin[(p + 1) & 1], lqb);
+      ctx->stream = main;
+      GPX_TRY(r);
+    }
+    const double* Sp = Sin + p * 5 * sqa;
+    const double* Tp = Tin[p & 1];
+    for (int q = 0; q < 7; ++q) {
+      const SProd& in = kStrassen[q];
+      const double* Aq = in.a < 0 ? Sp + (-1 - in.a) * sqa : (in.a == 0 ? Ap : Ap + qm * lap + qk);
+      const double* Bq = in.b < 0 ? Tp + (-1 - in.b) * sqb : (in.b == 0 ? Bp : Bp + qk * lbp + qn);
+      SDest sub2[GPX_MULTI_MAX];
+      int n2 = 0;
+      for (int d = 0; d < ns; ++d)
+        for (int j = 0; j < in.nq; ++j) sub2[n2++] = SDest{sub[d].c + qoff2[in.q[j]], sub[d].s * in.s[j]};
+      GPX_TRY(strassen_rec(ctx, Aq, in.a < 0 ? lqa : lap, Bq, in.b < 0 ? lqb : lbp, sub2, n2, ldc, qm, qn, qk, 0, nullptr));
+    }
+    if (p + 1 < 7) GPX_TRY(gpx_ov_fork(ctx, side, main));
+  }
+  return 0;
+}
+
 int launch_dist2_update(gpx_ctx* ctx, double* C, int64_t ldc, int64_t lr0, int64_t m, int64_t lc0, int64_t n, int64_t nb, int Pr,
                         int Pc, int pr, int pc, int64_t piece_stride, int64_t dsz, int nseg, const double* const* g,
                         const int64_t* ks, int below_diag) {
diff --git a/gpexp_amd/csrc/gpx_internal.h b/gpexp_amd/csrc/gpx_internal.h
--- a/gpexp_amd/csrc/gpx_internal.h
+++ b/gpexp_amd/csrc/gpx_internal.h
@@ -122,6 +122,8 @@
   int pw_done;
   std::vector<hipEvent_t> la_events;
   hipEvent_t ev_side = nullptr;
+  std::vector<hipEvent_t> ov_events;
+  size_t ov_next = 0;
   int cus;
   std::multimap<int64_t, void*> pool;
   int64_t pool_bytes;
@@ -162,6 +164,8 @@
 
 int gpx_kparams_sets(gpx_ctx* ctx, KParams* kp, const gpx_mat* A, const gpx_mat* B = nullptr, const gpx_mat* C = nullptr);
 int gpx_dev_alloc(gpx_ctx* ctx, int64_t bytes, void** out);
+hipEvent_t gpx_ov_event(gpx_ctx* ctx);
+int gpx_ov_fork(gpx_ctx* ctx, hipStream_t from, hipStream_t to);
 void gpx_dev_release(gpx_ctx* ctx, void* p, int64_t bytes);
 int gpx_mat_new(gpx_ctx* ctx, int64_t rows, int64_t cols, int pad, gpx_mat** out);
 
@@ -209,6 +213,11 @@
                     int64_t m, int64_t n, int64_t k, bool bt, bool accumulate, bool lower, int tri);
 constexpr int GPX_STRASSEN_MAX_DEPTH = 2;
 int64_t gemm_strassen_scratch_bytes(int64_t m, int64_t n, int64_t k, int depth);
+int64_t gemm_strassen_left_bytes(int64_t m, int64_t k, int depth);
+int64_t gemm_strassen_right_bytes(int64_t n, int64_t k, int depth);
+int launch_strassen_left_sums(gpx_ctx* ctx, const double* A, int64_t lda, int64_t m, int64_t k, int depth, double* S);
+int launch_gemm_strassen_ahead(gpx_ctx* ctx, const double* A, int64_t lda, const double* B, int64_t ldb, double* C, int64_t ldc,
+                               int64_t m, int64_t n, int64_t k, int depth, const double* S, double* T, hipStream_t side);
 int launch_gemm_strassen(gpx_ctx* ctx, const double* A, int64_t lda, const double* B, int64_t ldb, double* C, int64_t ldc,
                          int64_t m, int64_t n, int64_t k, int depth, double* scratch, int64_t scratch_bytes);
 int launch_gemm_ksplit(gpx_ctx* ctx, const double* A, int64_t lda, const double* B, int64_t ldb, double* C, int64_t ldc,
@@ -246,7 +255,18 @@
 int64_t chol_binv_order(int64_t n);
 int64_t chol_binv_elems(int64_t n);
 int chol_binv_finish(gpx_ctx* ctx, gpx_mat* L, int64_t ib);
-int chol_trsm_left_oop(gpx_ctx* ctx, gpx_mat* L, double* B, int64_t ldb, double* W, int64_t ldw, int64_t m);
+struct TrsmColsums {
+  int64_t rows;
+  double* partial;
+  int done;
+};
+enum { GPX_OVERLAP_SUMS = 1, GPX_OVERLAP_COLSUMS = 2, GPX_OVERLAP_ALL = 3 };
+struct TrsmTune {
+  int64_t min_rows[2], min_cols[2];
+  int64_t scratch_cap;
+};
+int chol_trsm_left_oop(gpx_ctx* ctx, gpx_mat* L, double* B, int64_t ldb, double* W, int64_t ldw, int64_t m,
+                       TrsmColsums* colsums = nullptr, const TrsmTune* tune = nullptr);
 int chol_trsm_left_group(gpx_ctx* ctx, const double* Lg, int64_t ld, const double* invd, int64_t w, int64_t below, int64_t ib,
                          double* B, int64_t ldb, int64_t m, double* inv, double* tmp, double* W, int64_t ldw);
 int64_t chol_potrf_panel_width(int64_t n);
@@ -265,6 +285,10 @@
 int launch_colreduce(gpx_ctx* ctx, const double* B, int64_t ld, int64_t rows, int64_t pcols, const double* v,
                      double* out, double* d_partial, int subtract = 0);
 int64_t colreduce_partial_elems(int64_t rows, int64_t pcols);
+void colreduce_plan(int64_t rows, int64_t pcols, int64_t* chunk, int64_t* nchunk);
+int launch_colreduce_chunks(gpx_ctx* ctx, const double* B, int64_t ld, int64_t rows, int64_t pcols, int64_t c0, int64_t c1,
+                            double* d_partial);
+int launch_colreduce_final(gpx_ctx* ctx, const double* d_partial, int64_t rows, int64_t pcols, double* out);
 int launch_rowreduce(gpx_ctx* ctx, const double* B, int64_t ld, int64_t rows, int64_t cols, const double* v,
                      double* out, int weighted_squares = 0);
 int launch_sum(gpx_ctx* ctx, const double* x, int64_t n, double* d_out);
diff --git a/gpexp_amd/csrc/reduce.hip b/gpexp_amd/csrc/reduce.hip
--- a/gpexp_amd/csrc/reduce.hip
+++ b/gpexp_amd/csrc/reduce.hip
@@ -1,4 +1,5 @@
 #include "gpx_internal.h"
+#include <algorithm>
 
 namespace {
 
@@ -103,6 +104,33 @@
   return 0;
 }
 
+void colreduce_plan(int64_t rows, int64_t pcols, int64_t* chunk, int64_t* nchunk) { plan(rows, pcols, chunk, nchunk); }
+
+int launch_colreduce_chunks(gpx_ctx* ctx, const double* B, int64_t ld, int64_t rows, int64_t pcols, int64_t c0, int64_t c1,
+                            double* d_partial) {
+  int64_t chunk, nchunk;
+  plan(rows, pcols, &chunk, &nchunk);
+  GPX_ARG(nchunk * pcols <= colreduce_partial_elems(rows, pcols), "colreduce: partial-sum plan exceeds its own bound");
+  GPX_ARG(c0 >= 0 && c0 < c1 && c1 <= nchunk, "colreduce: chunk range outside the plan");
+  const int64_t rbase = c0 * chunk, r1 = std::min(rows, c1 * chunk);
+  ProfScope ps(ctx, GPX_PROF_REDUCE, 2.0 * (double)(r1 - rbase) * pcols, 8.0 * (double)(r1 - rbase) * pcols);
+  dim3 grid((unsigned)((pcols + 255) / 256), (unsigned)(c1 - c0));
+  hipLaunchKernelGGL(colreduce_kernel, grid, dim3(256), 0, ctx->stream, B + rbase * ld, ld, rows - rbase, chunk,
+                     (const double*)nullptr, d_partial + c0 * pcols, pcols);
+  GPX_HIP(hipGetLastError());
+  return 0;
+}
+
+int launch_colreduce_final(gpx_ctx* ctx, const double* d_partial, int64_t rows, int64_t pcols, double* out) {
+  int64_t chunk, nchunk;
+  plan(rows, pcols, &chunk, &nchunk);
+  ProfScope ps(ctx, GPX_PROF_REDUCE, 0.0, 8.0 * (double)nchunk * pcols);
+  hipLaunchKernelGGL(colreduce_final_kernel, dim3((unsigned)((pcols + 255) / 256)), dim3(256), 0, ctx->stream, d_partial, nchunk,
+                     pcols, out, 0);
+  GPX_HIP(hipGetLastError());
+  return 0;
+}
+
 namespace {
 
 __global__ __launch_bounds__(256) void rowreduce_kernel(const double* __restrict__ B, int64_t ld, int64_t cols,
diff --git a/gpexp_amd/device.py b/gpexp_amd/device.py
--- a/gpexp_amd/device.py
+++ b/gpexp_amd/device.py
@@ -715,3 +715,11 @@
 
 def dbg_gemm_strassen_depth(ctx, A, B, Cm, depth):
     check(ctx.lib.gpx_dbg_gemm_strassen_depth(ctx.h, A.h, B.h, Cm.h, int(depth)))
+
+
+def dbg_trsm_left_oop(ctx, L, B, W, min_rows, min_cols, scratch_cap=-1, sum_rows=0):
+    mr = (c_i64 * 2)(int(min_rows[0]), int(min_rows[1]))
+    mc = (c_i64 * 2)(int(min_cols[0]), int(min_cols[1]))
+    sums = np.empty((B.shape[1] + 127) // 128 * 128) if sum_rows > 0 else None
+    check(ctx.lib.gpx_dbg_trsm_left_oop(ctx.h, L.h, B.h, W.h, mr, mc, int(scratch_cap), int(sum_rows), dptr(sums)))
+    return sums
diff --git a/include/gpx_debug.h b/include/gpx_debug.h
--- a/include/gpx_debug.h
+++ b/include/gpx_debug.h
@@ -10,6 +10,8 @@
 int gpx_dbg_gemm_ksplit(gpx_ctx* ctx, const gpx_mat* A, const gpx_mat* B, gpx_mat* C, int mode, int parts);
 int gpx_dbg_gemm_strassen(gpx_ctx* ctx, const gpx_mat* A, const gpx_mat* B, gpx_mat* C);
 int gpx_dbg_gemm_strassen_depth(gpx_ctx* ctx, const gpx_mat* A, const gpx_mat* B, gpx_mat* C, int depth);
+int gpx_dbg_trsm_left_oop(gpx_ctx* ctx, gpx_mat* L, gpx_mat* B, gpx_mat* W, const int64_t* min_rows, const int64_t* min_cols,
+                          int64_t scratch_cap, int64_t sum_rows, double* colsums);
 int gpx_dbg_spin(gpx_ctx* ctx, int ms);
 int64_t gpx_dbg_guard_violations(gpx_ctx* ctx);
 int gpx_dbg_guard_selftest(gpx_ctx* ctx);
diff --git a/profiles/solve_overlap_trace.py b/profiles/solve_overlap_trace.py
--- /dev/null
+++ b/profiles/solve_overlap_trace.py
@@ -0,0 +1,49 @@
+#!/usr/bin/env python3
+import csv
+import json
+import sys
+
+
+def main():
+    path = sys.argv[1]
+    steps = int(sys.argv[2]) if len(sys.argv) > 2 else 4
+    rows = list(csv.DictReader(open(path)))
+    name_k = [k for k in rows[0] if k.lower() in ("kernel_name", "name")][0]
+    b_k = [k for k in rows[0] if k.lower().startswith("start")][0]
+    e_k = [k for k in rows[0] if k.lower().startswith("end")][0]
+    gemm, side = [], {"strassen_sums": [], "colreduce_kernel": [], "kfill_rectn": []}
+    for r in rows:
+        n, b, e = r[name_k], int(r[b_k]), int(r[e_k])
+        if "gemm_f64" in n:
+            gemm.append((b, e))
+        for s in side:
+            if s in n:
+                side[s].append((b, e))
+    gemm.sort()
+    merged = []
+    for b, e in gemm:
+        if merged and b <= merged[-1][1]:
+            merged[-1][1] = max(merged[-1][1], e)
+        else:
+            merged.append([b, e])
+    starts = [m[0] for m in merged]
+    import bisect
+
+    def inside(b, e):
+        tot, i = 0, max(bisect.bisect_right(starts, b) - 1, 0)
+        while i < len(merged) and merged[i][0] < e:
+            tot += max(0, min(e, merged[i][1]) - max(b, merged[i][0]))
+            i += 1
+        return tot
+
+    out = {"steps_traced": steps, "gemm_launches_per_step": len(gemm) / steps,
+           "gemm_ms_per_step": sum(e - b for b, e in gemm) / 1e6 / steps,
+           "gemm_union_ms_per_step": sum(e - b for b, e in merged) / 1e6 / steps}
+    for s, iv in side.items():
+        out[s] = {"launches_per_step": len(iv) / steps, "ms_per_step": sum(e - b for b, e in iv) / 1e6 / steps,
+                  "ms_inside_gemm_launches_per_step": sum(inside(b, e) for b, e in iv) / 1e6 / steps}
+    print(json.dumps(out, indent=1))
+
+
+if __name__ == "__main__":
+    main()
```

New measurement: 104,900 points/s. No clear change (-0.3%).
